# nh13/DWGSIM

Hardware: AMD Instinct MI355X
Metric: M read-pairs/sec (2x150 bp PE) (higher is better)
Workload: dtype u8

## Files before the change

### dwgsim_amd/api.py

```python
from __future__ import annotations
import ctypes as C
import os
import shlex
from dataclasses import dataclass, field

_HERE = os.path.dirname(os.path.abspath(__file__))
LIB_PATH = os.environ.get("DWGSIM_HIP_LIB") or os.path.join(_HERE, "libdwgsim_hip.so")

STREAM_BWA1, STREAM_BWA2, STREAM_BFAST = 0, 1, 2
STREAM_NAMES = {0: "bwa.read1.fastq", 1: "bwa.read2.fastq", 2: "bfast.fastq"}


class Params(C.Structure):
    _fields_ = [
        ("e_start", C.c_double * 2), ("e_end", C.c_double * 2),
        ("is_inner", C.c_int32), ("dist", C.c_int32), ("std_dev", C.c_double),
        ("N", C.c_int64), ("C", C.c_double), ("length", C.c_int32 * 2),
        ("mut_rate", C.c_double), ("mut_freq", C.c_double), ("indel_frac", C.c_double), ("indel_extend", C.c_double),
        ("indel_min", C.c_int32), ("rand_read", C.c_double), ("max_n", C.c_int32), ("data_type", C.c_int32),
        ("strandedness", C.c_int32), ("read_one_strand", C.c_int32), ("is_hap", C.c_int32), ("seed", C.c_int32),
        ("fixed_quality", C.c_int32), ("quality_std", C.c_double), ("reads_output_type", C.c_int32),
        ("output_type", C.c_int32), ("amplicons", C.c_int32), ("read_prefix", C.c_char_p), ("flow_order", C.c_char_p),
        ("use_base_error", C.c_int32),
    ]
# ... 165 lines not shown

def parse_flags(flags: str, lib=None) -> Params:
    p = default_params(lib)
    toks = shlex.split(flags)
    i = 0
    keep = []
    mut_input = None
    regions = None
    while i < len(toks):
        t = toks[i]
        def arg():
            nonlocal i
            i += 1
            return toks[i]
        if t == "-i": p.is_inner = 1
        elif t == "-d": p.dist = int(arg())
        elif t == "-s": p.std_dev = float(arg())
        elif t == "-N": p.N = int(arg()); p.C = -1
        elif t == "-C": p.C = float(arg()); p.N = -1
        elif t == "-1": p.length[0] = int(arg())
        elif t == "-2": p.length[1] = int(arg())
        elif t == "-e": p.e_start[0], p.e_end[0] = _error_rate(arg())
        elif t == "-E": p.e_start[1], p.e_end[1] = _error_rate(arg())
        elif t == "-r": p.mut_rate = float(arg())
        elif t == "-F": p.mut_freq = float(arg())
        elif t == "-R": p.indel_frac = float(arg())
        elif t == "-X": p.indel_extend = float(arg())
        elif t == "-I": p.indel_min = int(arg())
        elif t == "-c": p.data_type = int(arg())
        elif t == "-S": p.strandedness = int(arg())
        elif t == "-A": p.read_one_strand = int(arg())
        elif t == "-n": p.max_n = int(arg())
        elif t == "-y": p.rand_read = float(arg())
        elif t == "-f": keep.append(arg().encode()); p.flow_order = keep[-1]
        elif t == "-B": p.use_base_error = 1
        elif t == "-H": p.is_hap = 1
        elif t == "-z": p.seed = int(arg())
        elif t == "-M": p.output_type = int(arg())
        elif t == "-P": keep.append(arg().encode()); p.read_prefix = keep[-1]
        elif t == "-q": p.fixed_quality = ord(arg()[0])
        elif t == "-Q": p.quality_std = float(arg())
        elif t == "-o": p.reads_output_type = int(arg())
        elif t == "-a": p.amplicons = 1
        elif t == "-x": regions = arg()
        elif t in ("-m", "-b", "-v"): mut_input = ({"-b": 0, "-m": 1, "-v": 2}[t], arg())
        else:
            raise DwgsimError(f"option {t} is not on the accelerated path")
        i += 1
    p._keep = keep
    p._regions = regions
    p._mut_input = mut_input
    return p


def read_fasta(path: str):
    import numpy as np
    out = []
    name, chunks = None, []
    with open(path, "rb") as f:
        data = f.read()
    at = data.find(b">")
    while at >= 0:
        nl = data.find(b"\n", at)
        header = data[at + 1:] if nl < 0 else data[at + 1:nl]
        nxt = -1 if nl < 0 else data.find(b">", nl + 1)
        body = b"" if nl < 0 else (data[nl + 1:] if nxt < 0 else data[nl + 1:nxt])
        header = header.replace(b"\r", b"")
        name = header.split(b" ")[0].split(b"\t")[0].decode("latin-1")
        arr = np.frombuffer(body, dtype=np.uint8)
        keep = ((arr >= 65) & (arr <= 90)) | ((arr >= 97) & (arr <= 122)) | (arr == 45) | (arr == 46)
        out.append((name, np.ascontiguousarray(arr[keep])))
        at = nxt
    return out


@dataclass
class JobResult:
    streams: dict = field(default_factory=dict)
    mutations_txt: bytes = b""
    mutations_vcf: bytes = b""
    n_pairs: int = 0
    n_random: int = 0
    n_retries: int = 0
    kernel_ms: float = 0.0
    sim_kernel_ms: float = 0.0
    walk_ms: float = 0.0
    flow_cap_mult: int = 1


VCF_HEADER_POST = (
    b"##INFO=<ID=AF,Number=A,Type=Float,Description=\"Allele Frequency\">\n"
    b"##INFO=<ID=pl,Number=1,Type=Integer,Description=\"Phasing: 1 - HET contig 1, #2 - HET contig #2, 3 - HOM both contigs\">\n"
    b"##INFO=<ID=mt,Number=1,Type=String,Description=\"Variant Type: SUBSTITUTE/INSERT/DELETE\">\n"
    b"#CHROM\tPOS\tID\tREF\tALT\tQUAL\tFILTER\tINFO\n")


class Context:

    def __init__(self, params: Params, device: int = 0, lib=None):
        self.lib = lib or load()
        self.params = params
        err = C.c_int(0)
        self.h = self.lib.dwgsim_hip_create(C.byref(params), device, C.byref(err))
        if not self.h:
            raise DwgsimError(f"dwgsim_hip_create failed with code {err.value}" + (" (no HIP device? there is no CPU fallback)" if err.value == -2 else " (the library said why on stderr)"))
        for kv in os.environ.get("DWGSIM_HIP_DEBUG", "").split(","):
            if "=" in kv:
                self.lib.dwgsim_hip_debug_option(self.h, kv.split("=")[0].encode(), int(kv.split("=")[1]))

    def close(self):
        if self.h:
            self.lib.dwgsim_hip_destroy(self.h)
            self.h = None

    def __enter__(self):
        return self

    def __exit__(self, *a):
        self.close()

    def _chk(self, rc):
        if rc < 0:
            raise DwgsimError(f"error {rc}: {self.lib.dwgsim_hip_last_error(self.h).decode(errors='replace')}")
        return rc

    def add_contig(self, name: str, ascii_arr, contig_index: int) -> int:
        import numpy as np
        arr = np.ascontiguousarray(ascii_arr, dtype=np.uint8)
        return self._chk(self.lib.dwgsim_hip_add_contig(self.h, name.encode(), arr.ctypes.data_as(C.c_void_p), len(arr), contig_index))

    def drop_contig(self, cid: int):
        self._chk(self.lib.dwgsim_hip_drop_contig(self.h, cid))

    def add_contigs(self, contigs, first_index: int = 0, indices=None) -> int:
        import numpy as np
        n = len(contigs)
        arrs = [np.ascontiguousarray(a, dtype=np.uint8) for _, a in contigs]
        names = (C.c_char_p * n)(*[nm.encode() for nm, _ in contigs])
        ptrs = (C.c_void_p * n)(*[a.ctypes.data for a in arrs])
        lens = (C.c_int64 * n)(*[len(a) for a in arrs])
        idx = (C.c_uint32 * n)(*(indices if indices is not None else range(first_index, first_index + n)))
        return self._chk(self.lib.dwgsim_hip_add_contigs(self.h, n, names, ptrs, lens, idx))

    def mutate_async(self, cid: int):
        self._chk(self.lib.dwgsim_hip_mutate_async(self.h, cid))

    def mutate_wait(self, cid: int):
        self._chk(self.lib.dwgsim_hip_mutate_wait(self.h, cid))

    @staticmethod
    def _ranges(ranges):
        arr = (Range * len(ranges))()
        for k, (cid, first, n) in enumerate(ranges):
            arr[k].contig, arr[k].first_ii, arr[k].n_pairs = cid, first, n
        return arr

    def count_random_ranges(self, ranges, per_range: bool = False):
        n = C.c_uint64(0)
        per = (C.c_uint64 * len(ranges))() if per_range else None
        self._chk(self.lib.dwgsim_hip_count_random_ranges(self.h, self._ranges(ranges), len(ranges), C.byref(n), per))
        return list(per) if per_range else n.value

    def simulate_ranges_async(self, ranges, rand_base: int = RAND_CHAIN, slot: int = 0):
        self._chk(self.lib.dwgsim_hip_simulate_ranges_async(self.h, self._ranges(ranges), len(ranges), rand_base, slot))

    def simulate_ranges(self, ranges, rand_base: int, slot: int = 0) -> Batch:
# ... 150 lines not shown
            if have_regions and not last_takes_rest:
                l_eff = ctx.region_length(ci, arr)
                if l_eff < 0:
                    continue
            n_pairs = pairs_for_contig(params, l_eff, tot_len, n_ref == 0, n_sim, lib)
            if n_pairs < 0:
                continue
        n_sim += n_pairs
        yield ci, name, arr, n_pairs, l_eff


def split_ranges(ranges, batch_pairs):
    batch, room = [], batch_pairs
    for cid, first, n in ranges:
        while n > 0:
            take = min(n, room)
            batch.append((cid, first, take))
            first += take; n -= take; room -= take
            if room == 0:
                yield batch
                batch, room = [], batch_pairs
    if batch:
        yield batch


def run_job(params: Params, contigs, device: int = 0, batch_pairs: int = 1 << 22, fetch: bool = True, lib=None, debug_options=None, group_bp: int = 0, check_list_form: bool = False) -> JobResult:
    lib = lib or load()
    res = JobResult(streams={0: bytearray(), 1: bytearray(), 2: bytearray()})
    want_mut = params.output_type != 1
    want_reads = params.output_type != 2
    vcf = bytearray()
    txt = bytearray()
    if want_mut:
        vcf += b"##fileformat=VCFv4.1\n"
        for name, arr in contigs:
            vcf += f"##contig=<ID={name},length={len(arr)}>\n".encode()
        vcf += VCF_HEADER_POST
    n_sim = 0
    rand_ii = 0
    with Context(params, device, lib) as ctx:
        for k, v in (debug_options or {}).items():
            ctx.debug_option(k, v)
        if getattr(params, "_mut_input", None):
            ctx.set_mutation_input(params._mut_input[0], params._mut_input[1], contigs)
        have_regions = bool(getattr(params, "_regions", None))
        sched = list(schedule_contigs(params, contigs, ctx, lib))
        groups, cur, cur_bp = [], [], 0
        for ent in sched:
            if cur and (group_bp <= 0 or cur_bp + len(ent[2]) > group_bp):
                groups.append(cur); cur, cur_bp = [], 0
            cur.append(ent); cur_bp += len(ent[2])
        if cur:
            groups.append(cur)
        for grp in groups:
            h0 = ctx.add_contigs([(name, arr) for _, name, arr, _, _ in grp], indices=[ci for ci, _, _, _, _ in grp])
            if have_regions:
                for k, ent in enumerate(grp):
                    ctx.set_placement_length(h0 + k, ent[4])
            ctx.mutate(h0)
            if want_mut:
                for k in range(len(grp)):
                    t, v = ctx.mutations_text(h0 + k)
                    txt += t
                    vcf += v
                if check_list_form:
                    tv = ctx.mutations_via_list(h0)
                    if b"".join(a for a, _ in tv) != b"".join(ctx.mutations_text(h0 + k)[0] for k in range(len(grp))) or \
                       b"".join(b for _, b in tv) != b"".join(ctx.mutations_text(h0 + k)[1] for k in range(len(grp))):
                        raise DwgsimError("mutations_take / mutlist_text differs from mutations_text")
            ranges = [(h0 + k, 0, ent[3]) for k, ent in enumerate(grp) if want_reads and ent[3] > 0]
            for batch in split_ranges(ranges, batch_pairs):
                b = ctx.simulate_ranges(batch, rand_ii, 0)
                res.kernel_ms += b.kernel_ms
                res.sim_kernel_ms += b.sim_kernel_ms
                res.n_retries += b.n_retries
                if fetch:
                    for s in range(3):
                        if b.bytes[s]:
                            res.streams[s] += ctx.fetch(0, s, b.bytes[s])
                rand_ii += b.n_random
                n_sim += b.n_pairs
            ctx.drop_contig(h0)
        res.flow_cap_mult = ctx.debug_get("flow_cap_mult")
    res.n_pairs = n_sim
    res.n_random = rand_ii
    res.mutations_txt = bytes(txt)
    res.mutations_vcf = bytes(vcf)
    res.streams = {k: bytes(v) for k, v in res.streams.items()}
    return res


def run_job_api(params: Params, contigs, devices=None, gzip_on_gpu: bool = True, batch_pairs: int = 0, group_bp: int = 0, min_share: int = 0,
                lib=None, keep_output: bool = True, offset_sink: bool = False) -> JobResult:
    import gzip as _gz
    import numpy as np
    lib = lib or load()
    res = JobResult(streams={0: bytearray(), 1: bytearray(), 2: bytearray()})
    raw = {0: [], 1: [], 2: []}
    txt, vcf = bytearray(), bytearray()
    if params.output_type != 1:
        vcf += b"##fileformat=VCFv4.1\n"
        for name, arr in contigs:
            vcf += f"##contig=<ID={name},length={len(arr)}>\n".encode()
        vcf += VCF_HEADER_POST
    order = {"mut": [], "text_n": {0: 0, 1: 0, 2: 0}}

    def on_mut(user, name, t, tl, v, vl):
        order["mut"].append(name.decode())
        txt.extend(C.string_at(t, tl) if tl else b"")
        vcf.extend(C.string_at(v, vl) if vl else b"")
        return 0

    def on_reads(user, stream, data, n, text_n, gz):
        order["text_n"][stream] += text_n
        if keep_output:
            raw[stream].append((bool(gz), C.string_at(data, n), text_n))
        return 0

    import threading
    at_lock = threading.Lock(); at_pieces = {0: [], 1: [], 2: []}; at_threads = set()

    def on_reads_at(user, stream, offset, data, n, text_n, gz):
        blob = C.string_at(data, n) if keep_output else b""
        with at_lock:
            at_threads.add(threading.get_ident())
            order["text_n"][stream] += text_n
            at_pieces[stream].append((offset, n, bool(gz), blob, text_n))
        return 0

    sink = JobSink(None, MUT_CB(on_mut), READS_CB(on_reads), MSG_CB(lambda u, m: None), READS_AT_CB(on_reads_at) if offset_sink else READS_AT_CB())
    opt = JobOptions(1 if gzip_on_gpu else 0, 1, batch_pairs, group_bp, min_share)
    err = C.c_int(0)
    devs = (C.c_int * len(devices))(*devices) if devices else None
    job = lib.dwgsim_hip_job_create(C.byref(params), devs, len(devices) if devices else 0, C.byref(sink), C.byref(opt), C.byref(err))
    if not job:
        raise DwgsimError(f"dwgsim_hip_job_create failed with code {err.value}")
    try:
        def chk(rc):
            if rc < 0:
                raise DwgsimError(f"error {rc}: {lib.dwgsim_hip_job_last_error(job).decode(errors='replace')}")
        n = len(contigs)
        names = (C.c_char_p * n)(*[nm.encode() for nm, _ in contigs])
        lens = (C.c_int64 * n)(*[len(a) for _, a in contigs])
        chk(lib.dwgsim_hip_job_set_contig_table(job, names, lens, n))
        if getattr(params, "_regions", None):
            chk(lib.dwgsim_hip_job_set_regions(job, params._regions.encode()))
        if getattr(params, "_mut_input", None):
            chk(lib.dwgsim_hip_job_set_mutation_input(job, params._mut_input[0], params._mut_input[1].encode()))
        chk(lib.dwgsim_hip_job_prepare(job, None))
        for name, arr in contigs:
            a = np.ascontiguousarray(arr, dtype=np.uint8)
            r = lib.dwgsim_hip_job_add_contig(job, name.encode(), a.ctypes.data_as(C.c_void_p), len(a))
            if r < 0 and not is_skip(r):
                chk(r)
            if r > 0:
                res.n_pairs += r
        chk(lib.dwgsim_hip_job_finish(job))
    finally:
        lib.dwgsim_hip_job_destroy(job)
    if offset_sink:
        for s_ in range(3):
            at = 0
            for off, n, gz, blob, text_n in sorted(at_pieces[s_]):
                if off != at:
                    raise DwgsimError(f"reads_at: stream {s_} has a gap or an overlap at offset {at} (next piece at {off})")
                at += n
# ... 176 lines not shown
```

### dwgsim_amd/csrc/dw_host.cpp

```cpp
#include <hip/hip_runtime.h>
#include <math.h>
#include <stdio.h>
#include <stdlib.h>
#include <string.h>
#include <limits.h>
#include <ctype.h>
#include <stdarg.h>
#include <stdint.h>
#include <sys/mman.h>
#include <mutex>
#include <thread>
#include <string>
#include <vector>
#include <algorithm>
#include <array>
#include <stddef.h>
#include <type_traits>
#include "../../include/dwgsim_hip.h"
#include "dw_kernels.hpp"
#include "dw_launch.hpp"
#include "dw_mutin.hpp"
#include "dw_mem.hpp"

using namespace dw;

namespace {

struct HostIns { std::vector<int32_t> pos; std::vector<uint32_t> len, off; std::vector<uint8_t> bases; };

struct Member {
    std::string name;
    int64_t l = 0, l_place = 0;
    uint32_t contig_index = 0;
    int32_t start = 0;
    int32_t reg_off = 0, n_reg = 0;
    uint32_t name_off = 0; int32_t name_fixed_len = 0;
    ResolvedContig rc;
};

struct GroupMem {
    DevMem d_ref, d_cells[2], d_view[2];
    DevMem d_ins_pos[2], d_ins_len[2], d_ins_off[2], d_ins_bases[2];
    DevMem d_names, d_reg, d_seg;
    std::vector<uint8_t> h_names; std::vector<int32_t> h_reg, h_seg;
    DevMem d_summ[2], d_summ2[2];
    DevMem d_refview, d_refsumm, d_refsumm2, d_dirty;
    DevEvent ev_walk, ev_walk0;
    HostMem h_wc;
};

struct WalkCounters {
    uint64_t unused0[7];
    uint64_t n_cand;
    uint32_t max_del;
    struct { uint32_t entries, bases; } ins[2];
    uint32_t unused1;
    uint32_t slot_over;
    uint32_t n_cand_true;
    uint64_t mut_debug[2];
    uint64_t n_listed;
    uint64_t unused2;
};
static_assert(std::is_standard_layout<WalkCounters>::value && sizeof(WalkCounters) == 16 * 8, "the walk's counter block is 16 u64 words");
static_assert(offsetof(WalkCounters, n_cand) == 7 * 8 && offsetof(WalkCounters, max_del) == 8 * 8 && offsetof(WalkCounters, ins) == 8 * 8 + 4 && offsetof(WalkCounters, slot_over) == 8 * 8 + 6 * 4 &&
              offsetof(WalkCounters, n_cand_true) == 8 * 8 + 7 * 4 && offsetof(WalkCounters, mut_debug) == 12 * 8 && offsetof(WalkCounters, n_listed) == 14 * 8, "every counter at the word the kernels were given before the block had a type");
struct WcSpan { size_t off, bytes; };
#define WC_SPAN(first, last) WcSpan{offsetof(WalkCounters, first), offsetof(WalkCounters, last) + sizeof(WalkCounters::last) - offsetof(WalkCounters, first)}
constexpr WcSpan WC_RANDOM = WC_SPAN(n_cand, n_cand_true), WC_FILE = WC_SPAN(mut_debug, mut_debug), WC_LISTED = WC_SPAN(n_listed, n_listed);

struct Group {
    bool alive = false, mutated = false, walk_pending = false;
    int first_handle = -1;
    std::vector<Member> m;
    int64_t total = 0;
    GroupMem mem;
    uint32_t n_ins[2] = {0, 0}, n_ins_bases[2] = {0, 0};
    int fixed_max = 0;
    uint32_t n_cand = 0;
    bool dirty_any = false, dirty_all = false;
    int walk_attempt = 0; uint32_t walk_cap = 0; size_t walk_cap_bases = 0; bool walk_reset = false;
    uint32_t n_patch = 0, n_patch_ev = 0;
    bool list_valid = false; std::vector<int32_t> pos; std::vector<uint32_t> cells; HostIns ins[2];
};

struct HandleRef { int group = -1, k = 0; };

constexpr int N_COUNTERS = 32;

struct Counters {
    DevMem d; HostMem h;
    uint64_t *dev() const { return d.get<uint64_t>(); }
    uint64_t *host() const { return h.get<uint64_t>(); }
};

struct Slot {
    Counters counters;
    hipEvent_t ev_k0 = nullptr, ev_k1 = nullptr, ev_end = nullptr, ev_done = nullptr, ev_fetched = nullptr;
    bool pending = false, empty = true, fetch_in_flight = false;
    int group = -1;
    uint64_t n_pairs = 0, out_bytes[3] = {0, 0, 0}, gz_bytes[3] = {0, 0, 0};
    DevMem gz_out[3], gz_status, segs;
    HostMem h_segs;
    std::vector<dwgsim_hip_range_t> ranges;
    DevMem d_rerun_chain;
    int cap_mult = 1;
};

}

struct dwgsim_hip_ctx {
    dwgsim_hip_params_t prm;
    std::string read_prefix;
    std::vector<uint8_t> flow;
    DevMem d_flow;
    int device = 0;
    hipStream_t stream = nullptr;
    hipStream_t copy_stream = nullptr;
    hipStream_t walk_stream = nullptr;
    hipStream_t count_stream = nullptr;
    std::string err;
    double e_by[2] = {0, 0};
    DevMem d_thr[2];
    DevMem d_thr32[2]; int e_full = 0;
    DevMem d_qbase[2]; int32_t qb_words = 1;
    DevMem d_rand_fixed; int32_t rand_fixed_len = 0;
    std::vector<Group> groups;
    std::vector<GroupMem> pool;
    std::vector<HandleRef> handles;
    DevMem meta, fail_summ, block_rand, status_all, out[DWGSIM_HIP_SLOTS][3], split_state, split_hand, split_agg, split_pre, split_chunk;
    DevMem w_slots, w_slot_aux;
    int site_slots = -1; int64_t site_slot_cap = -1;
    DevMem scratch_mask, scratch_cnt, scratch_status, w_cand, w_ev, w_flags, w_lo, w_sufmin, w_bound, w_ppos, w_pcells, up_ascii, l_pos, l_cells, place_segs, place_rand, place_list, place_aux;
    HostMem h_up; hipEvent_t ev_up = nullptr; bool up_in_flight = false;
    HostMem h_place_segs, h_range_rand;
    std::vector<int32_t> h_ppos; std::vector<uint16_t> h_pcells; std::vector<Event> h_pev;
    bool seq_justify = false, dense_view = false;
    MutInput mutin; bool has_mutin = false;
    Regions regions; bool has_regions = false;
    DevMem flow_scratch, flow_free;
    Counters counters;
    DevMem d_wcounters;
    Counters pcounters;
    Slot slot[DWGSIM_HIP_SLOTS];
    DevMem d_chain;
    int chain_contig = -1; uint64_t chain_next_ii = 0;
    bool has_carry_override = false; uint64_t carry_override = 0;
    int flow_cap_forced = 0;
    int flow_cap_mult = 1;
    int ion_lds = -1;
    int n_cu = 0; int flow_slots = 0;
    int64_t walk_cap = -1; bool phases = false; int writer = -1, force_threads = 0; int64_t place_cap = -1; uint64_t place_open = 0; double walk_us = 0, count_us = 0; int split = -1;
    int64_t sim_form = 0;
    int64_t walk_form = 0;
    hipEvent_t ev_cnt0 = nullptr, ev_cnt1 = nullptr;
    bool gzip_on = false; DevMem d_crc_table, d_crc_shift;
    HostMem h_stage;
    std::string txt, vcf;
};

namespace {

#define HIPC(ctx, call) do { hipError_t e_ = (call); if (e_ != hipSuccess) { char b_[512]; snprintf(b_, sizeof b_, "HIP error %s at %s:%d (%s)", hipGetErrorString(e_), __FILE__, __LINE__, #call); (ctx)->err = b_; return DWGSIM_HIP_ERR_DEVICE; } } while (0)

hipError_t dev_malloc(dwgsim_hip_ctx *c, void **p, size_t bytes)
{
    hipError_t e = DevKind::alloc(p, bytes);
    if (e == hipSuccess || c->pool.empty()) return e;
    (void)hipGetLastError();
    hipStreamSynchronize(c->walk_stream);
    c->pool.clear();
    return DevKind::alloc(p, bytes);
}

hipError_t reserve(dwgsim_hip_ctx *c, DevMem &b, size_t need, size_t want)
{
    return b.reserve(need, want, [c](void **p, size_t n) { return dev_malloc(c, p, n); });
}

int ensure(dwgsim_hip_ctx *c, DevMem &b, size_t bytes)
{
    HIPC(c, reserve(c, b, bytes, bytes + bytes / 8 + 4096));
    return 0;
}

int upload(dwgsim_hip_ctx *c, DevMem &b, const void *src, size_t n)
{
    HIPC(c, reserve(c, b, n, n));
    const hipError_t e = hipMemcpy(b.get(), src, n, hipMemcpyHostToDevice);
    if (e != hipSuccess) b.reset();
    HIPC(c, e);
    return 0;
}

template <class T> int upload_table(dwgsim_hip_ctx_t *c, DevMem &d, const std::vector<T> &h, size_t slack)
{
    HIPC(c, reserve(c, d, sizeof(T) * h.size(), sizeof(T) * (h.size() + slack)));
    HIPC(c, hipMemcpyAsync(d.get(), h.data(), sizeof(T) * h.size(), hipMemcpyHostToDevice, c->walk_stream));
    return 0;
}

uint8_t nt4(int ch)
{
    switch (ch) { case 'A': case 'a': return 0; case 'C': case 'c': return 1; case 'G': case 'g': return 2; case 'T': case 't': return 3; case '-': return 5; default: return 4; }
}

void lazy_quality_params(double sigma, float *k, float *eps, float *lmin, int32_t *near1_zero)
{
    const double two_ln2 = 2.0 * log(2.0);
    double lm = 0.98 * (0.45 / sigma) * (0.45 / sigma) / two_ln2;
    if (!(lm < 0x1p-4)) lm = 0x1p-4;
    *near1_zero = lm >= 0x1p-10 ? 1 : 0;
    if (lm < 0x1p-10) lm = 0x1p-10;
    *lmin = (float)lm;
    lm = (double)*lmin * (1.0 - 0x1p-20);
    *k = (float)(sqrt(two_ln2) * sigma);
    *eps = (float)(1.5 * sigma * (3.4e-7 / sqrt(lm) + 7.2e-6) + 0x1p-18);
}

WalkParams walk_params(const dwgsim_hip_ctx *c)
{
    WalkParams w; w.mut_rate = c->prm.mut_rate; w.indel_frac = c->prm.indel_frac; w.indel_extend = c->prm.indel_extend;
    w.indel_min = c->prm.indel_min; w.is_hap = c->prm.is_hap; w.seed = (uint32_t)c->prm.seed;
    w.mut_thr = !(c->prm.mut_rate > 0) ? 0 : c->prm.mut_rate >= 1.0 ? 0x100000000ull : (uint64_t)ceil(c->prm.mut_rate * 4294967296.0);
    flow_gap_params(w.mut_thr, &w.gap_r, &w.gap_s);
    w.lg = reinterpret_cast<const uint32_t *>(c->d_flow.get() + 64);
    return w;
}

size_t padded_cells(const Group &g) { return (size_t)g.total + CELL_PAD; }

size_t view_bytes(size_t padded) { return padded / 2; }
size_t summ_bytes(size_t padded) { return sizeof(uint16_t) * (padded / SUMM_CELLS); }
size_t summ2_bytes(size_t padded) { return sizeof(uint16_t) * (padded / SUMM2_CELLS); }
uint32_t dirty_words(size_t padded) { return (uint32_t)((padded + 32 * SUMM_CELLS - 1) / (32 * SUMM_CELLS)); }
// ... 476 lines not shown
    const size_t view = view_bytes(padded) + 32, summ = summ_bytes(padded) + 32, summ2 = summ2_bytes(padded) + 32;
    const struct { DevMem *buf; size_t bytes; } cellbufs[] = {
        {&M.d_ref, padded}, {&M.d_cells[0], padded}, {&M.d_view[0], view}, {&M.d_summ[0], summ}, {&M.d_summ2[0], summ2},
        {&M.d_cells[1], padded}, {&M.d_view[1], view}, {&M.d_summ[1], summ}, {&M.d_summ2[1], summ2},
        {&M.d_refview, view}, {&M.d_refsumm, summ}, {&M.d_refsumm2, summ2}, {&M.d_dirty, dirty_bytes(padded)}};
    for (const auto &b : cellbufs) b.buf->reset();
    for (const auto &b : cellbufs) HIPC(c, reserve(c, *b.buf, b.bytes, b.bytes));
    return 0;
}

static int upload_sequence(dwgsim_hip_ctx_t *c, int n, const uint8_t *const *ascii, const int64_t *lens, const int64_t *starts, int64_t total, size_t padded, bool &must_wait)
{
    if (ensure(c, c->up_ascii, padded)) return DWGSIM_HIP_ERR_DEVICE;
    uint8_t *d_ascii = c->up_ascii.get();
    must_wait = true;
    bool laid_out = true;
    for (int k = 0; k < n && laid_out; ++k) if (lens[k] > 0 && ascii[k] != ascii[0] + starts[k]) laid_out = false;
    if (laid_out && n > 0 && ascii[0] && is_page_locked(ascii[0])) {
        HIPC(c, hipMemcpyAsync(d_ascii, ascii[0], (size_t)total, hipMemcpyHostToDevice, c->walk_stream));
        HIPC(c, hipMemsetAsync(d_ascii + total, 0, padded - (size_t)total, c->walk_stream));
        must_wait = false;
    } else if (n <= 8) {
        HIPC(c, hipMemsetAsync(d_ascii, 0, padded, c->walk_stream));
        for (int k = 0; k < n; ++k) if (lens[k] > 0) HIPC(c, hipMemcpyAsync(d_ascii + starts[k], ascii[k], (size_t)lens[k], hipMemcpyHostToDevice, c->walk_stream));
    } else {
        if (c->up_in_flight) { HIPC(c, hipEventSynchronize(c->ev_up)); c->up_in_flight = false; }
        HIPC(c, c->h_up.reserve((size_t)total, (size_t)total + (size_t)total / 4 + 4096));
        uint8_t *h_up = c->h_up.get();
        for (int k = 0; k < n; ++k) {
            const int64_t end = starts[k] + lens[k], next = k + 1 < n ? starts[k + 1] : total;
            if (lens[k] > 0) memcpy(h_up + starts[k], ascii[k], (size_t)lens[k]);
            memset(h_up + end, 0, (size_t)(next - end));
        }
        HIPC(c, hipMemcpyAsync(d_ascii, h_up, (size_t)total, hipMemcpyHostToDevice, c->walk_stream));
        HIPC(c, hipMemsetAsync(d_ascii + total, 0, padded - (size_t)total, c->walk_stream));
        HIPC(c, hipEventRecord(c->ev_up, c->walk_stream)); c->up_in_flight = true;
    }
    return 0;
}

static int make_pristine(dwgsim_hip_ctx_t *c, const Group &g)
{
    const GroupMem &M = g.mem;
    const int64_t n_cells = (int64_t)padded_cells(g) & ~(int64_t)15;
    uint8_t *ref = M.d_ref.get();
    launch_pack(c->walk_stream, c->up_ascii.get(), ref, M.d_cells[0].get(), M.d_cells[1].get(), n_cells);
    launch_make_view(c->walk_stream, ref, ref, n_cells, g.total, M.d_refview.get(), M.d_view[0].get(), M.d_refsumm.get<uint16_t>(), M.d_summ[0].get<uint16_t>(), M.d_refsumm2.get<uint16_t>(), M.d_summ2[0].get<uint16_t>());
    if (const int rc = restore_pristine(c, g, 1, R_VIEW | R_SUMM | R_SUMM2, c->walk_stream)) return rc;
    if (const int rc = clear_dirty(c, g, c->walk_stream)) return rc;
    HIPC(c, hipGetLastError());
    return 0;
}

static int upload_group_tables(dwgsim_hip_ctx_t *c, Group &g)
{
    GroupMem &M = g.mem;
    const int n = (int)g.m.size();
    M.h_seg.assign((size_t)(3 * n + 1), 0);
    for (int k = 0; k < n; ++k) { M.h_seg[(size_t)k] = g.m[(size_t)k].start; M.h_seg[(size_t)(n + 1 + k)] = (int32_t)g.m[(size_t)k].l; M.h_seg[(size_t)(2 * n + 1 + k)] = (int32_t)g.m[(size_t)k].contig_index; }
    M.h_seg[(size_t)n] = (int32_t)g.total;
    if (const int rc = upload_table(c, M.d_seg, M.h_seg, 64)) return rc;
    M.h_names.clear();
    for (Member &m : g.m) {
        const std::string nf = c->read_prefix.empty() ? m.name : c->read_prefix + "_" + m.name;
        m.name_fixed_len = (int32_t)nf.size(); m.name_off = (uint32_t)M.h_names.size();
        if (m.name_fixed_len > g.fixed_max) g.fixed_max = m.name_fixed_len;
        const size_t room = ((nf.size() + 1 < 256 ? 272 : nf.size() + 1 + 16) + 15) & ~(size_t)15;
        M.h_names.resize(M.h_names.size() + room, 0);
        M.h_names[m.name_off] = '@'; memcpy(&M.h_names[m.name_off + 1], nf.data(), nf.size());
    }
    if (const int rc = upload_table(c, M.d_names, M.h_names, 4096)) return rc;
    M.h_reg.clear();
    if (!c->has_regions) return 0;
    for (Member &m : g.m) {
        std::vector<int32_t> st, en; int64_t tot = 0;
        for (size_t q = 0; q < c->regions.contig.size(); ++q) if (c->regions.contig[q] == m.contig_index) { st.push_back((int32_t)c->regions.start[q]); en.push_back((int32_t)c->regions.end[q]); tot += c->regions.end[q] - c->regions.start[q]; }
        m.reg_off = (int32_t)M.h_reg.size(); m.n_reg = (int32_t)st.size(); m.l_place = tot;
        M.h_reg.insert(M.h_reg.end(), st.begin(), st.end()); M.h_reg.insert(M.h_reg.end(), en.begin(), en.end());
    }
    M.h_reg.push_back(0);
    return upload_table(c, M.d_reg, M.h_reg, 64);
}

static int build_group(dwgsim_hip_ctx_t *c, Group &g, const uint8_t *const *ascii, const int64_t *lens, const int64_t *starts)
{
    const int n = (int)g.m.size();
    const size_t padded = padded_cells(g);
    bool must_wait = true;
    if (const int rc = reserve_cell_buffers(c, g.mem, padded)) return rc;
    if (const int rc = upload_sequence(c, n, ascii, lens, starts, g.total, padded, must_wait)) return rc;
    if (const int rc = make_pristine(c, g)) return rc;
    if (const int rc = upload_group_tables(c, g)) return rc;
    if (c->has_mutin) for (int k = 0; k < n; ++k) resolve_mutation_input(c->mutin, g.m[(size_t)k].contig_index, ascii[k], lens[k], (uint32_t)c->prm.seed, c->prm.is_hap != 0, g.m[(size_t)k].rc);
    if (must_wait) HIPC(c, hipStreamSynchronize(c->walk_stream));
    return 0;
}

int dwgsim_hip_add_contigs(dwgsim_hip_ctx_t *c, int n, const char *const *names, const uint8_t *const *ascii, const int64_t *lens, const uint32_t *contig_index)
{
    if (!c || n < 1 || !names || !ascii || !lens || !contig_index) { if (c) c->err = "bad contig arguments"; return DWGSIM_HIP_ERR_ARG; }
    for (int k = 0; k < n; ++k) if (!names[k] || (!ascii[k] && lens[k] > 0) || lens[k] < 0 || lens[k] > INT32_MAX) { c->err = "bad contig arguments"; return DWGSIM_HIP_ERR_ARG; }
    std::vector<int64_t> starts((size_t)n);
    const int64_t total = dwgsim_hip_group_layout(lens, n, starts.data());
    if (total < 0 || total > (int64_t)INT32_MAX - 2 * GROUP_ALIGN) { c->err = "dwgsim-hip: the contigs of one group must stay below 2^31 cells in all (add them in smaller groups)\n"; return DWGSIM_HIP_ERR_ARG; }
    HIPC(c, hipSetDevice(c->device));
    const int gid = take_group(c, (size_t)total + CELL_PAD);
    Group &g = c->groups[(size_t)gid];
    g.alive = true; g.total = total; g.first_handle = (int)c->handles.size();
    g.m.resize((size_t)n);
    for (int k = 0; k < n; ++k) { Member &m = g.m[(size_t)k]; m.name = names[k]; m.l = m.l_place = lens[k]; m.contig_index = contig_index[k]; m.start = (int32_t)starts[(size_t)k]; }
    const int rc = build_group(c, g, ascii, lens, starts.data());
    if (rc != 0) { (void)hipStreamSynchronize(c->walk_stream); g = Group(); return rc; }
    for (int k = 0; k < n; ++k) c->handles.push_back(HandleRef{gid, k});
    return g.first_handle;
}

int dwgsim_hip_add_contig(dwgsim_hip_ctx_t *c, const char *name, const uint8_t *ascii, int64_t len, uint32_t contig_index)
{
    return dwgsim_hip_add_contigs(c, 1, &name, &ascii, &len, &contig_index);
}

int dwgsim_hip_drop_contig(dwgsim_hip_ctx_t *c, int contig)
{
    Group *g = get_group(c, contig);
    if (!g) return DWGSIM_HIP_ERR_ARG;
    hipSetDevice(c->device);
    const int gid = (int)(g - c->groups.data());
    for (int s = 0; s < DWGSIM_HIP_SLOTS; ++s) if (c->slot[s].pending && !c->slot[s].empty && c->slot[s].group == gid) { c->err = "drop_contig: a batch that reads this group has not been waited for (dwgsim_hip_wait first)"; return DWGSIM_HIP_ERR_STATE; }
    if (g->walk_pending) hipEventSynchronize(g->mem.ev_walk.get());
    for (size_t k = 0; k < g->m.size(); ++k) { if (c->chain_contig == g->first_handle + (int)k) c->chain_contig = -1; c->handles[(size_t)g->first_handle + k].group = -1; }
    c->pool.push_back(std::move(g->mem));
    *g = Group();
    if (c->pool.size() > 3) {
        hipStreamSynchronize(c->walk_stream);
        c->pool.erase(c->pool.begin());
    }
    return DWGSIM_HIP_OK;
}

int dwgsim_hip_set_regions(dwgsim_hip_ctx_t *c, const char *path, const char *const *names, const int64_t *lens, int n_contigs, uint64_t *total_len)
{
    if (!c || !path || n_contigs < 0 || (n_contigs && (!names || !lens))) { if (c) c->err = "bad regions arguments"; return DWGSIM_HIP_ERR_ARG; }
    if (c->prm.amplicons) { c->err = "Error: cannot use a regions BED file (-x) when simulating amplicons (-a)\n"; return DWGSIM_HIP_ERR_ARG; }
    std::vector<ContigName> tab;
    for (int i = 0; i < n_contigs; ++i) tab.push_back(ContigName{names[i], lens[i]});
    std::string err;
    if (!parse_regions(path, tab, c->regions, err)) { c->err = err; c->has_regions = false; return DWGSIM_HIP_ERR_ARG; }
    c->has_regions = true;
    uint64_t tot = 0;
    for (size_t q = 0; q < c->regions.start.size(); ++q) tot += c->regions.end[q] - c->regions.start[q];
    if (total_len) *total_len = tot;
    return DWGSIM_HIP_OK;
}

int64_t dwgsim_hip_contig_region_length(dwgsim_hip_ctx_t *c, uint32_t contig_index, const uint8_t *ascii, int64_t len, int64_t *non_acgt, int64_t *region_bases)
{
    if (non_acgt) *non_acgt = 0;
    if (region_bases) *region_bases = len;
    if (!c || !c->has_regions) return len;
    int64_t m = 0, num_n = 0;
    for (size_t q = 0; q < c->regions.contig.size(); ++q) if (c->regions.contig[q] == contig_index) {
        m += c->regions.end[q] - c->regions.start[q];
        for (int64_t p = c->regions.start[q]; p <= (int64_t)c->regions.end[q]; ++p) { const int ch = (p >= 1 && p - 1 < len) ? ascii[p - 1] : 'N'; if (nt4(ch) >= 4) ++num_n; }
    }
    if (non_acgt) *non_acgt = num_n;
    if (region_bases) *region_bases = m;
    if (m == 0) return DWGSIM_HIP_SKIP_NO_REGION;
    if (0.95 < num_n / (double)m) return DWGSIM_HIP_SKIP_NON_ACGT;
    return m;
}

int dwgsim_hip_contig_set_placement_length(dwgsim_hip_ctx_t *c, int contig, int64_t l)
{
    int k = 0;
    Group *g = get_group(c, contig, &k);
// ... 79 lines not shown
        HIPC(c, hipMemcpyAsync(c->w_pcells.get(), c->h_pcells.data(), sizeof(uint16_t) * np, hipMemcpyHostToDevice, st));
        if (nev) HIPC(c, hipMemcpyAsync(c->w_ev.get(), c->h_pev.data(), sizeof(Event) * nev, hipMemcpyHostToDevice, st));
        launch_apply_patches(st, c->w_ppos.get<int32_t>(), c->w_pcells.get<uint16_t>(), np, M.d_cells[0].get(), M.d_cells[1].get());
        launch_mut_debug(st, M.d_ref.get(), M.d_cells[0].get(), M.d_cells[1].get(), g.total, &wc->mut_debug[0]);
        if (nev) justify(c, st, c->w_ev.get<Event>(), Count{nullptr, nev}, group_dev(g));
        launch_mut_debug(st, M.d_ref.get(), M.d_cells[0].get(), M.d_cells[1].get(), g.total, &wc->mut_debug[1]);
    }
    make_views(st, g);
    g.dirty_all = true;
    HIPC(c, hipGetLastError());
    HIPC(c, wc_fetch(c, M, WC_FILE, st));
    HIPC(c, hipEventRecord(M.ev_walk.get(), st));
    return DWGSIM_HIP_OK;
}

enum class Restore { None, Chunks, All };
struct WalkPlan {
    uint32_t cap; size_t ncap, cap_bases;
    uint32_t nblk;
    bool use_slots; uint32_t nbs, slot_cap; size_t slot_bytes;
    Restore restore;
    bool dense;
};

static WalkPlan walk_plan(const dwgsim_hip_ctx_t *c, const Group &g)
{
    WalkPlan P;
    P.cap = g.walk_cap; P.ncap = P.cap ? P.cap : 1; P.cap_bases = g.walk_cap_bases;
    P.nblk = (uint32_t)((g.total + SCAN_POS_PER_BLOCK - 1) / SCAN_POS_PER_BLOCK);
    P.nbs = site_scan_blocks(g.total);
    const double m = (double)site_scan_block_positions() * (c->prm.mut_rate > 0 ? c->prm.mut_rate : 0.0);
    P.slot_cap = (uint32_t)std::min<double>((double)site_scan_block_positions(), m + 8.0 * sqrt(m + 1.0) + 32.0);
    if (c->site_slot_cap >= 0) P.slot_cap = (uint32_t)std::max<int64_t>(1, c->site_slot_cap);
    P.slot_bytes = (size_t)P.nbs * P.slot_cap * sizeof(int32_t);
    P.use_slots = g.walk_attempt == 0 && c->site_slots != 0 && P.nbs > 0 && (c->site_slots > 0 || P.slot_bytes <= std::max<size_t>((size_t)64 << 20, P.ncap * 16));
    P.restore = g.walk_attempt > 0 || g.dirty_all ? Restore::All : g.dirty_any ? Restore::Chunks : Restore::None;
    P.dense = c->seq_justify || c->dense_view;
    return P;
}

static int walk_reserve(dwgsim_hip_ctx_t *c, Group &g, const WalkPlan &P)
{
    if (ensure(c, c->scratch_status, ((size_t)P.nblk + 2) * sizeof(uint64_t)) ||
        ensure(c, c->w_cand, sizeof(int32_t) * P.ncap) || ensure(c, c->w_ev, sizeof(Event) * P.ncap) ||
        ensure(c, c->w_flags, sizeof(uint4) * (P.ncap + 64)) ||
        ensure(c, c->w_lo, sizeof(int32_t) * P.ncap) || ensure(c, c->w_sufmin, sizeof(int32_t) * (P.ncap + 64)) ||
        ensure(c, c->w_bound, P.ncap)) return DWGSIM_HIP_ERR_DEVICE;
    for (int h = 0; h < 2; ++h) if (const int rc = ensure_ins(c, g, h, P.ncap, P.cap_bases)) return rc;
    if (P.use_slots && (ensure(c, c->w_slots, P.slot_bytes) || ensure(c, c->w_slot_aux, 2 * (size_t)P.nbs * sizeof(uint32_t)))) return DWGSIM_HIP_ERR_DEVICE;
    return DWGSIM_HIP_OK;
}

static int walk_launch(dwgsim_hip_ctx_t *c, Group &g, const WalkPlan &P)
{
    hipStream_t st = c->walk_stream;
    const WalkParams wp = walk_params(c);
    const SegTab seg = seg_tab(g);
    const GroupMem &M = g.mem;
    WalkCounters *wc = c->d_wcounters.get<WalkCounters>();
    int32_t *d_cand = c->w_cand.get<int32_t>(); Event *d_ev = c->w_ev.get<Event>(); uint4 *d_flags = c->w_flags.get<uint4>();
    uint32_t *tot4 = &wc->ins[0].entries;
    const Count nc{&wc->n_cand, P.cap};
    HIPC(c, wc_fill(c, WC_RANDOM, 0, st));
    if (P.use_slots) launch_site_scan_slots(st, M.d_refview.get(), g.total, seg, wp, c->w_slots.get<int32_t>(), P.slot_cap, c->w_slot_aux.get<uint32_t>(), d_cand, P.cap, &wc->n_cand, &wc->slot_over);
    else {
        uint64_t *d_status = c->scratch_status.get<uint64_t>();
        HIPC(c, hipMemsetAsync(d_status, 0, ((size_t)P.nblk + 2) * sizeof(uint64_t), st));
        launch_site_scan_list(st, M.d_refview.get(), g.total, seg, wp, d_status, d_status + P.nblk, d_cand, P.cap, &wc->n_cand);
    }
    launch_events(st, d_cand, nc, M.d_ref.get(), seg, wp, d_ev, &wc->max_del);
    launch_resolve(st, d_ev, nc, &wc->max_del, d_flags, tot4);
    ContigDev cd = group_dev(g);
    cd.tot4 = tot4; cd.cap_bases[0] = (uint32_t)std::min<size_t>(ins_bases_cap(g, 0), 0xFFFFFFFFu); cd.cap_bases[1] = (uint32_t)std::min<size_t>(ins_bases_cap(g, 1), 0xFFFFFFFFu);
    launch_apply(st, d_ev, nc, d_flags, cd, wp);
    justify(c, st, d_ev, nc, cd);
    if (P.dense) {
        make_views(st, g);
        g.dirty_all = true;
    } else {
        launch_mark_dirty(st, d_ev, nc, c->w_lo.get<int32_t>(), M.d_dirty.get<uint32_t>());
        dirty_chunks(st, false, g);
        g.dirty_any = true;
    }
    HIPC(c, hipGetLastError());
    return DWGSIM_HIP_OK;
}

static int walk_random(dwgsim_hip_ctx_t *c, Group &g)
{
    const WalkPlan P = walk_plan(c, g);
    if (const int rc = walk_reserve(c, g, P)) return rc;
    c->walk_form = pack_walk_form(g.walk_attempt, false, P.use_slots, (int)P.restore, P.dense);
    hipStream_t st = c->walk_stream;
    HIPC(c, hipEventRecord(g.mem.ev_walk0.get(), st));
    if (P.restore == Restore::All) { for (int h = 0; h < 2; ++h) if (const int rc = restore_pristine(c, g, h, R_ALL, st)) return rc; }
    else if (P.restore == Restore::Chunks) dirty_chunks(st, true, g);
    if (P.restore != Restore::None) { if (const int rc = clear_dirty(c, g, st)) return rc; g.dirty_all = g.dirty_any = false; }
    if (const int rc = walk_launch(c, g, P)) return rc;
    HIPC(c, wc_fetch(c, g.mem, WC_RANDOM, st));
    HIPC(c, hipEventRecord(g.mem.ev_walk.get(), st));
    return DWGSIM_HIP_OK;
}

static void collect_file_mutations(dwgsim_hip_ctx_t *c, const Group &g, HostIns (&hi)[2])
{
    c->h_ppos.clear(); c->h_pcells.clear(); c->h_pev.clear();
    for (size_t k = 0; k < g.m.size(); ++k) {
        const Member &m = g.m[k];
        for (size_t q = 0; q < m.rc.pos.size(); ++q) {
            c->h_ppos.push_back(m.rc.pos[q] + m.start); c->h_pcells.push_back(m.rc.cells[q]);
            if (m.rc.cells[q] & 0x3030) { Event e; e.pos = m.rc.pos[q] + m.start; e.type = 4; e.hap = 3; e.base = 0; e.live = 1; e.len = 1; e.seg = (uint32_t)k; c->h_pev.push_back(e); }
        }
        for (int h = 0; h < 2; ++h) for (const InsPayload &ip : m.rc.ins[h]) {
            hi[h].pos.push_back(ip.pos + m.start); hi[h].len.push_back((uint32_t)ip.bases.size()); hi[h].off.push_back((uint32_t)hi[h].bases.size());
            hi[h].bases.insert(hi[h].bases.end(), ip.bases.begin(), ip.bases.end());
        }
    }
}

static int upload_ins_tables(dwgsim_hip_ctx_t *c, Group &g, HostIns (&hi)[2])
{
    for (int h = 0; h < 2; ++h) {
        const size_t n = hi[h].pos.size(), nb = hi[h].bases.size();
        g.n_ins[h] = (uint32_t)n; g.n_ins_bases[h] = (uint32_t)nb;
        if (const int rc = ensure_ins(c, g, h, n ? n : 1, nb ? nb : 1)) return rc;
        if (n) for (const InsTable &t : ins_tables(g.mem, h, hi[h])) HIPC(c, hipMemcpy(t.dev, t.host, t.bytes, hipMemcpyHostToDevice));
    }
    return DWGSIM_HIP_OK;
}

static void initial_walk_caps(const dwgsim_hip_ctx_t *c, Group &g)
{
    double mean = 0;
    for (const Member &m : g.m) mean += (double)m.l * c->prm.mut_rate;
    g.walk_cap = (uint32_t)std::min<double>((double)g.total, mean + 8.0 * sqrt(mean + 1.0) + 256.0);
    g.walk_cap_bases = (size_t)g.walk_cap * 8 + 4096;
    if (c->walk_cap >= 0) { g.walk_cap = (uint32_t)c->walk_cap; g.walk_cap_bases = 1; }
}

int dwgsim_hip_mutate_async(dwgsim_hip_ctx_t *c, int contig)
{
    Group *gp = get_group(c, contig);
    if (!gp) return DWGSIM_HIP_ERR_ARG;
    Group &g = *gp;
    if (g.walk_pending) { c->err = "mutate: the group's previous walk was not waited for"; return DWGSIM_HIP_ERR_STATE; }
    for (const Slot &sl : c->slot) if (sl.pending && sl.group == c->handles[(size_t)contig].group) { c->err = "mutate: a batch that reads this group is still in flight (wait for it first)"; return DWGSIM_HIP_ERR_STATE; }
    HIPC(c, hipSetDevice(c->device));
    g.walk_reset = g.mutated;
    for (int h = 0; h < 2; ++h) g.n_ins[h] = g.n_ins_bases[h] = 0;
    g.mutated = true; g.n_cand = 0; g.list_valid = false;
    g.walk_attempt = 0;
    if (g.total == 0) return DWGSIM_HIP_OK;
    if (c->has_mutin) {
        HIPC(c, hipStreamSynchronize(c->walk_stream));
        HostIns hi[2];
        collect_file_mutations(c, g, hi);
        g.n_patch = (uint32_t)c->h_ppos.size(); g.n_patch_ev = (uint32_t)c->h_pev.size();
        g.n_cand = g.n_patch_ev;
        HIPC(c, hipStreamSynchronize(c->walk_stream));
        if (const int rc = upload_ins_tables(c, g, hi)) return rc;
    } else initial_walk_caps(c, g);
    if (const int rc = c->has_mutin ? walk_file_driven(c, g) : walk_random(c, g)) return rc;
    g.walk_pending = true;
    return DWGSIM_HIP_OK;
}

// ... 189 lines not shown
    if (const int rc = fetch_mutated_list(c, g)) return rc;
    const Member &m = g.m[(size_t)km];
    format_mutations(ListView{g.pos.data(), g.cells.data(), g.pos.size(), g.ins}, m.name, m.start, m.l, c->txt, c->vcf);
    if (txt) *txt = c->txt.data();
    if (txt_len) *txt_len = c->txt.size();
    if (vcf) *vcf = c->vcf.data();
    if (vcf_len) *vcf_len = c->vcf.size();
    return DWGSIM_HIP_OK;
}

struct dwgsim_hip_mutlist {
    std::vector<int32_t> pos; std::vector<uint32_t> cells; HostIns ins[2];
    struct M { std::string name; int64_t l; int32_t start; };
    std::vector<M> m;
    std::string txt, vcf;
};

dwgsim_hip_mutlist_t *dwgsim_hip_mutations_take(dwgsim_hip_ctx_t *c, int contig, int *n_contigs)
{
    if (n_contigs) *n_contigs = 0;
    if (!c) return nullptr;
    Group *gp = get_group(c, contig);
    if (!gp) return nullptr;
    Group &g = *gp;
    if (!g.mutated || g.walk_pending) { c->err = "mutate_contig must run first"; return nullptr; }
    if (hipSetDevice(c->device) != hipSuccess) { c->err = "mutations_take: device error"; return nullptr; }
    if (fetch_mutated_list(c, g)) return nullptr;
    auto *L = new dwgsim_hip_mutlist();
    L->pos.swap(g.pos); L->cells.swap(g.cells);
    for (int h = 0; h < 2; ++h) { L->ins[h] = std::move(g.ins[h]); g.ins[h] = HostIns(); }
    g.list_valid = false;
    for (const Member &m : g.m) L->m.push_back({m.name, m.l, m.start});
    if (n_contigs) *n_contigs = (int)L->m.size();
    return L;
}

int dwgsim_hip_mutlist_text(dwgsim_hip_mutlist_t *L, int k, const char **txt, size_t *txt_len, const char **vcf, size_t *vcf_len)
{
    if (!L || k < 0 || k >= (int)L->m.size()) return DWGSIM_HIP_ERR_ARG;
    const auto &m = L->m[(size_t)k];
    format_mutations(ListView{L->pos.data(), L->cells.data(), L->pos.size(), L->ins}, m.name, m.start, m.l, L->txt, L->vcf);
    if (txt) *txt = L->txt.data();
    if (txt_len) *txt_len = L->txt.size();
    if (vcf) *vcf = L->vcf.data();
    if (vcf_len) *vcf_len = L->vcf.size();
    return DWGSIM_HIP_OK;
}

void dwgsim_hip_mutlist_free(dwgsim_hip_mutlist_t *L) { delete L; }

namespace {
struct Launch { SimForm f; SimArgs a; Group *g = nullptr; std::vector<SimSeg> segs; uint64_t n_pairs = 0; uint32_t nblk = 0; int fixed_max = 0; };
struct SimPlan {
    size_t cap[3];
    int32_t lb_shift; bool too_many;
    size_t block_rand, status, meta, fail_summ, split_state, split_hand, split_agg, split_pre, split_chunk;
    bool scratch; int32_t flow_slots; size_t flow_scratch, flow_free;
    size_t segs, gz_chunks[3], gz_cap[3], gz_status;
};
struct ChainSet { uint64_t *words; int set_rand, set_carry; uint64_t carry; };
}

static int build_ranges(dwgsim_hip_ctx_t *c, const dwgsim_hip_range_t *r, int n, uint64_t ppb, Launch &L)
{
    if (!r || n < 1) { c->err = "bad range arguments"; return DWGSIM_HIP_ERR_ARG; }
    Group *g = nullptr;
    uint64_t pairs = 0, blocks = 0; int fmax = 0;
    std::vector<SimSeg> &segs = L.segs;
    segs.clear();
    for (int q = 0; q < n; ++q) {
        int k = 0;
        Group *gq = get_group(c, r[q].contig, &k);
        if (!gq) return DWGSIM_HIP_ERR_ARG;
        if (g && gq != g) { c->err = "the ranges of one call must belong to contigs that were added together (dwgsim_hip_add_contigs)"; return DWGSIM_HIP_ERR_ARG; }
        g = gq;
        if (r[q].n_pairs == 0) continue;
        const Member &m = g->m[(size_t)k];
        if (c->has_regions && m.n_reg == 0 && c->prm.rand_read < 1.0) { c->err = "dwgsim-hip: this contig has no target region (-x): the reference's placement loop would not terminate\n"; return DWGSIM_HIP_ERR_ARG; }
        SimSeg s; memset(&s, 0, sizeof s);
        s.first_block = (uint32_t)blocks; s.contig_index = m.contig_index; s.start = m.start; s.l = (int32_t)m.l;
        s.first_ii = r[q].first_ii; s.n_pairs = r[q].n_pairs; s.pair_off = pairs; s.l_place = m.l_place;
        s.reg_off = m.reg_off; s.n_reg = m.n_reg; s.name_off = m.name_off; s.name_fixed_len = m.name_fixed_len;
        s.contig_start = r[q].first_ii == 0 ? 1u : 0u;
        segs.push_back(s);
        pairs += r[q].n_pairs; blocks += (r[q].n_pairs + ppb - 1) / ppb;
        if (m.name_fixed_len > fmax) fmax = m.name_fixed_len;
        if (blocks > 0x7fffffffull) { c->err = "too many pairs in one call"; return DWGSIM_HIP_ERR_ARG; }
    }
    if (!g->mutated || g->walk_pending) { c->err = "mutate_contig must run first"; return DWGSIM_HIP_ERR_STATE; }
    L.g = g; L.n_pairs = pairs; L.nblk = (uint32_t)blocks; L.fixed_max = fmax;
    return DWGSIM_HIP_OK;
}

static int sim_form(dwgsim_hip_ctx_t *c, SimForm &f)
{
    const dwgsim_hip_params_t &p = c->prm;
    const size_t qb = (size_t)c->qb_words;
    const int lmax = p.length[0] > p.length[1] ? p.length[0] : p.length[1];
    f = SimForm();
    f.lpp = p.length[1] > 0 ? 2 : 1;
    f.out = (p.reads_output_type != 2 ? 1 : 0) | (p.reads_output_type != 1 ? 2 : 0);
    f.dt = p.data_type;
    f.nthr = SIM_THREADS;
    f.cap = lmax; f.lds_words = (lmax + 7) / 8;
    bool fifo = true;
    if (p.data_type == 0) {
        const int cap_fifo = 5, cap_reg = (p.reads_output_type == 0) ? 4 : 5;
        const int b_fifo = sim_blocks_per_cu(sim_lds_bytes((size_t)f.lds_words, SIM_THREADS, qb, true), cap_fifo), b_reg = sim_blocks_per_cu(sim_lds_bytes((size_t)f.lds_words, SIM_THREADS, qb, false), cap_reg);
        if (b_fifo < b_reg && !(p.reads_output_type == 0 && b_fifo >= 3)) fifo = false;
        if (c->writer >= 0) fifo = c->writer != 0;
    }
    const size_t need = sim_lds_bytes((size_t)f.lds_words, SIM_THREADS, qb, fifo);
    if (p.data_type != 2 && (need > SIM_LDS_BUDGET || ((sim_blocks_per_cu(need, 8) < 2 || c->force_threads == SIM_THREADS_LONG) && c->force_threads != SIM_THREADS))) {
        f.nthr = SIM_THREADS_LONG; fifo = true;
        if (sim_lds_bytes(0, SIM_THREADS_LONG, qb, true) > SIM_LDS_BUDGET) {
            char b[160]; snprintf(b, sizeof b, "dwgsim-hip: reads longer than %d bases are not supported for -c 0 / -c 1\n", (int)((SIM_LDS_BUDGET - SIM_THREADS_LONG * SIM_FIFO_BYTES) / 2 - 16));
            c->err = b; return DWGSIM_HIP_ERR_UNSUP;
        }
    }
    if (p.data_type == 2) {
        f.cap = std::max(flow_base_capacity(c), lmax) * c->flow_cap_mult;
        f.lds_words = (f.cap + 15) / 16; f.cap = 16 * f.lds_words;
        f.stack_words = std::min(FLOW_STACK_WORDS * c->flow_cap_mult, FLOW_STACK_WORDS_MAX);
        const size_t per_lane = (size_t)(f.lds_words + f.stack_words);
        const size_t need256 = sim_lds_bytes(per_lane, SIM_THREADS, qb, true), need64 = sim_lds_bytes(per_lane, ION_THREADS_SMALL, qb, true);
        int mode = c->ion_lds;
        if (mode < 0) mode = (need256 <= SIM_LDS_BUDGET && sim_blocks_per_cu(need256, 8) >= 2) ? 1 : (need64 <= SIM_LDS_BUDGET && sim_blocks_per_cu(need64, 32) >= 4) ? 2 : 0;
        if ((mode == 1 && need256 > SIM_LDS_BUDGET) || (mode == 2 && need64 > SIM_LDS_BUDGET)) mode = 0;
        f.dt = mode != 0 ? 3 : 2; f.nthr = mode == 2 ? ION_THREADS_SMALL : SIM_THREADS;
    }
    const bool split_wins = lmax <= 50;
    f.split = (p.data_type == 0 && f.nthr == SIM_THREADS && (c->split < 0 ? split_wins : c->split != 0)) ? 1 : 0;
    if (f.dt == 3 && f.nthr == SIM_THREADS && f.cap < 32768 && c->split != 0) f.split = 1;
    if (f.split && c->writer < 0) fifo = true;
    const size_t stage = f.dt == 3 ? (size_t)(f.lds_words + f.stack_words) : f.dt == 2 ? (size_t)f.stack_words : f.nthr != SIM_THREADS ? 0 : (size_t)f.lds_words;
    if (f.split) { f.wr = fifo ? 2 : 0; f.lds = sim_lds_bytes(stage, (size_t)f.nthr, 0, false); f.lds_b = sim_lds_bytes(0, (size_t)f.nthr, qb, fifo, SIM_FIFO_BYTES_WIDE); }
    else { f.wr = fifo ? 1 : 0; f.lds = sim_lds_bytes(stage, (size_t)f.nthr, qb, fifo); }
    return 0;
}

static void fill_sim_args(const dwgsim_hip_ctx_t *c, const Group &g, const SimForm &f, SimArgs &a)
{
    const dwgsim_hip_params_t &p = c->prm;
    memset(&a, 0, sizeof a);
    a.p.std_dev = p.std_dev; a.p.mut_freq = p.mut_freq; a.p.rand_read = p.rand_read; a.p.quality_std = p.quality_std;
    a.p.dist = p.dist; a.p.is_inner = p.is_inner; a.p.len[0] = p.length[0]; a.p.len[1] = p.length[1]; a.p.max_n = p.max_n;
    a.p.strandedness = p.strandedness; a.p.read_one_strand = p.read_one_strand; a.p.amplicons = p.amplicons;
    a.p.fixed_quality = p.fixed_quality; a.p.data_type = p.data_type;
    a.p.has_bfast = p.reads_output_type != 1; a.p.has_bwa = p.reads_output_type != 2;
    a.p.seed = (uint32_t)p.seed;
    lazy_quality_params(p.quality_std, &a.p.q_k, &a.p.q_eps, &a.p.q_lmin, &a.p.q_near1);
    fill_haps(g, a.hap);
    a.chain = c->d_chain.get<uint64_t>();
    a.have_regions = c->has_regions ? 1 : 0; a.reg = g.mem.d_reg.get<int32_t>();
    for (int j = 0; j < 2; ++j) { a.e_thr[j] = c->d_thr[j].get<uint64_t>(); a.e_thr32[j] = c->d_thr32[j].get<uint32_t>(); a.qbase[j] = c->d_qbase[j].get<uint32_t>() ? c->d_qbase[j].get<uint32_t>() : c->d_qbase[0].get<uint32_t>(); }
    a.qb_words = c->qb_words;
    a.e_full = c->e_full;
    a.names = g.mem.d_names.get();
    a.summ[0] = g.mem.d_summ[0].get<uint16_t>(); a.summ[1] = g.mem.d_summ[1].get<uint16_t>(); a.summ2[0] = g.mem.d_summ2[0].get<uint16_t>(); a.summ2[1] = g.mem.d_summ2[1].get<uint16_t>();
    a.place_fast = (!c->has_regions && !p.amplicons && p.std_dev * 12.1 + 2.0 < 1e9) ? 1 : 0;
    a.place_k = a.place_fast ? (int32_t)ceil(p.std_dev * 12.1) + 2 : 0;
    a.rand_fixed = c->d_rand_fixed.get(); a.rand_fixed_len = c->rand_fixed_len;
    a.sim_threads = f.nthr; a.fifo = f.wr != 0; a.split = f.split; a.ion_lds = f.dt == 3;
    a.cap = f.cap; a.lds_words = f.lds_words; a.flow_stack_words = f.stack_words;
    a.flow = c->d_flow.get(); a.flow_len = (int32_t)c->flow.size();
    for (int j = 0; j < 2; ++j) {
        const int n = c->prm.length[j];
        uint64_t tmax = 0, tmin = ~0ull;
        for (int i = 0; i < n; ++i) {
            const double ei = c->prm.e_start[j] + c->e_by[j] * i;
            const uint64_t t = !(ei > 0) ? 0 : ei >= 1.0 ? 0x100000000ull : (uint64_t)ceil(ei * 4294967296.0);
            tmax = std::max(tmax, t); tmin = std::min(tmin, t);
        }
        a.err_thr_max[j] = n > 0 ? tmax : 0; a.err_ramp[j] = (n > 0 && tmin != tmax) ? 1 : 0;
        flow_gap_params(a.err_thr_max[j], &a.err_gap_r[j], &a.err_gap_s[j]);
    }
    for (int j = 0; j < 2; ++j) {
        const double e0 = c->prm.e_start[j];
        flow_gap_params(!(e0 > 0) ? 0 : e0 >= 1.0 ? 0x100000000ull : (uint64_t)ceil(e0 * 4294967296.0), &a.flow_gap_r[j], &a.flow_gap_s[j]);
    }
}

static int sim_resolve(dwgsim_hip_ctx_t *c, const dwgsim_hip_range_t *r, int n, Launch &L)
{
    if (!r || n < 1) { c->err = "bad range arguments"; return DWGSIM_HIP_ERR_ARG; }
    if (!get_group(c, r[0].contig)) return DWGSIM_HIP_ERR_ARG;
    if (const int rc = sim_form(c, L.f)) return rc;
    if (const int rc = build_ranges(c, r, n, (uint64_t)(L.f.nthr / L.f.lpp), L)) return rc;
    fill_sim_args(c, *L.g, L.f, L.a);
    return DWGSIM_HIP_OK;
}

int dwgsim_hip_count_random_ranges(dwgsim_hip_ctx_t *c, const dwgsim_hip_range_t *r, int n, uint64_t *n_random, uint64_t *per_range)
{
    if (!c) return DWGSIM_HIP_ERR_ARG;
    if (n_random) *n_random = 0;
    if (per_range) for (int q = 0; q < n; ++q) per_range[q] = 0;
    Launch L;
    if (const int rc = build_ranges(c, r, n, PLACE_PAIRS, L)) return rc;
    const uint64_t n_pairs = L.n_pairs; const uint32_t n_blocks = L.nblk;
    if (n_pairs == 0) return DWGSIM_HIP_OK;
    Group &g = *L.g;
    HIPC(c, hipSetDevice(c->device));
    hipStream_t st = c->count_stream;
    if (g.walk_pending) { if (const int rc = dwgsim_hip_mutate_wait(c, g.first_handle)) return rc; }
    if (g.mem.ev_walk.get() && g.mutated) HIPC(c, hipStreamWaitEvent(st, g.mem.ev_walk.get(), 0));
    if (const int rc = sim_form(c, L.f)) return rc;
    SimArgs &a = L.a; fill_sim_args(c, g, L.f, a);
    const size_t ns = L.segs.size();
    if (ensure(c, c->place_rand, sizeof(uint32_t) * ((size_t)n_blocks + 1)) || ensure(c, c->place_segs, sizeof(SimSeg) * ns) ||
        ensure(c, c->place_aux, PLACE_LISTS * 16 * sizeof(uint32_t) + sizeof(uint64_t) * ns)) return DWGSIM_HIP_ERR_DEVICE;
    if (sizeof(SimSeg) * ns > c->h_place_segs.cap() || sizeof(uint64_t) * ns > c->h_range_rand.cap()) HIPC(c, hipStreamSynchronize(st));
    HIPC(c, c->h_place_segs.reserve(sizeof(SimSeg) * ns, sizeof(SimSeg) * (ns + 64))); HIPC(c, c->h_range_rand.reserve(sizeof(uint64_t) * ns, sizeof(uint64_t) * (ns + 64)));
    const uint64_t *h_range_rand = c->h_range_rand.get<uint64_t>();
    memcpy(c->h_place_segs.get(), L.segs.data(), sizeof(SimSeg) * ns);
    HIPC(c, hipMemcpyAsync(c->place_segs.get(), c->h_place_segs.get(), sizeof(SimSeg) * ns, hipMemcpyHostToDevice, st));
    a.segs = c->place_segs.get<SimSeg>(); a.n_seg = (int32_t)ns; a.n_blocks = n_blocks; a.n_pairs = n_pairs;
    a.block_rand = c->place_rand.get<uint32_t>(); a.counters = c->pcounters.dev();
    const uint64_t waves = (uint64_t)n_blocks * (PLACE_PAIRS / 64);
    const uint32_t cap_full = (uint32_t)((waves + PLACE_LISTS - 1) / PLACE_LISTS) * 64u;
    uint32_t cap = (uint32_t)std::min<uint64_t>(cap_full, 1024 + n_pairs / PLACE_LISTS / 8);
    if (c->place_cap >= 0 && (uint64_t)c->place_cap < cap) cap = (uint32_t)c->place_cap;
    for (int attempt = 0;; ++attempt) {
        if (ensure(c, c->place_list, sizeof(uint32_t) * (size_t)cap * PLACE_LISTS)) return DWGSIM_HIP_ERR_DEVICE;
        a.place_list = c->place_list.get<uint32_t>(); a.place_list_cap = cap;
        a.place_list_n = c->place_aux.get<uint32_t>(); a.range_rand = reinterpret_cast<uint64_t *>(c->place_aux.get<uint8_t>() + PLACE_LISTS * 16 * sizeof(uint32_t));
        HIPC(c, hipMemsetAsync(c->pcounters.dev(), 0, N_COUNTERS * sizeof(uint64_t), st));
        HIPC(c, hipMemsetAsync(c->place_aux.get(), 0, PLACE_LISTS * 16 * sizeof(uint32_t) + sizeof(uint64_t) * ns, st));
        HIPC(c, hipEventRecord(c->ev_cnt0, st));
        launch_place(st, a);
        HIPC(c, hipEventRecord(c->ev_cnt1, st));
        HIPC(c, hipGetLastError());
        HIPC(c, hipMemcpyAsync(c->pcounters.host(), c->pcounters.dev(), N_COUNTERS * sizeof(uint64_t), hipMemcpyDeviceToHost, st));
        HIPC(c, hipMemcpyAsync(c->h_range_rand.get(), a.range_rand, sizeof(uint64_t) * ns, hipMemcpyDeviceToHost, st));
        HIPC(c, hipStreamSynchronize(st));
        { float ms = 0; if (hipEventElapsedTime(&ms, c->ev_cnt0, c->ev_cnt1) == hipSuccess) c->count_us += 1e3 * ms; else (void)hipGetLastError(); }
        if (!(c->pcounters.host()[2] & 16) || attempt > 0) break;
        cap = cap_full;
    }
    if (c->pcounters.host()[2] & 16) { c->err = "count_random: the list of undecided pairs overflowed twice"; return DWGSIM_HIP_ERR_FAILED; }
    if (c->pcounters.host()[2]) { char b[128]; snprintf(b, sizeof b, "\r[dwgsim_core] failed to generate a read after %d trials\n", MAX_ATTEMPTS + 1); c->err = b; return DWGSIM_HIP_ERR_FAILED; }
    c->place_open = c->pcounters.host()[5];
// ... 101 lines not shown
    for (int j = 0; j < 4; ++j) a.status[j] = f.split ? nullptr : c->status_all.get<uint64_t>() + (size_t)j * (size_t)nblk;
    if (f.split) { a.split_state = c->split_state.get<uint32_t>(); a.split_hand = c->split_hand.get<uint32_t>(); a.split_agg = c->split_agg.get<uint32_t>(); a.split_pre = c->split_pre.get<uint64_t>(); a.split_chunk = c->split_chunk.get<uint64_t>(); }
    if (P.scratch) { a.flow_scratch = c->flow_scratch.get<uint32_t>(); a.flow_free = c->flow_free.get<uint64_t>(); a.flow_slots = P.flow_slots; }
    sl.group = c->handles[(size_t)L.g->first_handle].group;
    launch_init(c->stream, sl.counters.dev(), (uint32_t)N_COUNTERS, a.status[0], f.split ? 0 : 4 * (uint64_t)nblk, a.flow_free, a.flow_free ? 256 + 8 * (uint64_t)nblk : 0,
                ch.words, rand_base, ch.set_rand, ch.carry, ch.set_carry);
    HIPC(c, hipEventRecord(sl.ev_k0, c->stream));
    c->sim_form = (int64_t)f.nthr << 20 | f.lpp << 16 | f.out << 12 | f.dt << 8 | f.wr << 4 | f.split;
    if (!launch_simulate(c->stream, a, f)) { c->err = "simulate: no k_simulate instance for this form"; return DWGSIM_HIP_ERR_FAILED; }
    HIPC(c, hipEventRecord(sl.ev_k1, c->stream));
    sl.cap_mult = c->flow_cap_mult;
    if (!rerun) launch_failrule(c->stream, a.meta, n_pairs, opens, c->fail_summ.get<uint64_t>(), sl.counters.dev(), c->d_chain.get<uint64_t>());
    if (c->gzip_on) {
        HIPC(c, hipMemsetAsync(sl.gz_status.get(), 0, P.gz_status, c->stream));
        size_t off = 0;
        for (int t = 0; t < 3; ++t) {
            if (P.cap[t] == 0) continue;
            launch_gzip(c->stream, a.out[t], &sl.counters.dev()[4 + t], P.cap[t], sl.gz_out[t].get<uint8_t>(), P.gz_cap[t], sl.gz_status.get<uint64_t>() + off, &sl.counters.dev()[28 + t], &sl.counters.dev()[24 + t], &sl.counters.dev()[2],
                        c->d_crc_table.get<uint32_t>(), c->d_crc_shift.get<uint32_t>());
            off += P.gz_chunks[t];
        }
    }
    HIPC(c, hipEventRecord(sl.ev_end, c->stream));
    HIPC(c, hipGetLastError());
    HIPC(c, hipMemcpyAsync(sl.counters.host(), sl.counters.dev(), N_COUNTERS * sizeof(uint64_t), hipMemcpyDeviceToHost, c->stream));
    HIPC(c, hipEventRecord(sl.ev_done, c->stream));
    sl.pending = true;
    return DWGSIM_HIP_OK;
}

static int sim_enqueue(dwgsim_hip_ctx_t *c, const dwgsim_hip_range_t *r, int n, uint64_t rand_base, int slot, bool rerun)
{
    if (!c || slot < 0 || slot >= DWGSIM_HIP_SLOTS) { if (c) c->err = "bad simulate arguments"; return DWGSIM_HIP_ERR_ARG; }
    if (c->slot[slot].pending) { c->err = "simulate: the slot still holds a batch that was not waited for"; return DWGSIM_HIP_ERR_STATE; }
    Launch L;
    if (const int rc = sim_resolve(c, r, n, L)) return rc;
    HIPC(c, hipSetDevice(c->device));
    const SimPlan P = sim_plan(c, L);
    if (P.too_many) { c->err = "too many pairs in one call"; return DWGSIM_HIP_ERR_ARG; }
    if (L.n_pairs) { if (const int rc = sim_reserve(c, slot, P)) return rc; }
    return sim_launch(c, slot, L, P, sim_chain(c, c->slot[slot], r, n, rand_base != DWGSIM_HIP_RAND_CHAIN, rerun), rand_base, rerun);
}

int dwgsim_hip_simulate_ranges_async(dwgsim_hip_ctx_t *c, const dwgsim_hip_range_t *r, int n, uint64_t rand_base, int slot) { return sim_enqueue(c, r, n, rand_base, slot, false); }

int dwgsim_hip_simulate_async(dwgsim_hip_ctx_t *c, int contig, uint64_t first_ii, uint64_t n_pairs, uint64_t rand_base, int slot)
{
    dwgsim_hip_range_t r; memset(&r, 0, sizeof r); r.contig = contig; r.first_ii = first_ii; r.n_pairs = n_pairs;
    return dwgsim_hip_simulate_ranges_async(c, &r, 1, rand_base, slot);
}

int dwgsim_hip_wait(dwgsim_hip_ctx_t *c, int slot, dwgsim_hip_batch_t *out)
{
    if (!c || slot < 0 || slot >= DWGSIM_HIP_SLOTS) { if (c) c->err = "bad slot"; return DWGSIM_HIP_ERR_ARG; }
    Slot &sl = c->slot[slot];
    if (out) memset(out, 0, sizeof *out);
    if (sl.empty) { sl.pending = false; return DWGSIM_HIP_OK; }
    if (!sl.pending) { c->err = "wait: no batch was enqueued on this slot"; return DWGSIM_HIP_ERR_STATE; }
    HIPC(c, hipSetDevice(c->device));
    HIPC(c, hipEventSynchronize(sl.ev_done));
    sl.pending = false;
    uint64_t *h = sl.counters.host();
    if ((h[2] & 2) && !(h[2] & ~(2ull | 8ull)) && c->prm.data_type == 2) {
        uint64_t keep[8]; for (int q = 0; q < 6; ++q) keep[q] = h[16 + q];
        const uint64_t base = h[22];
        while (h[2] & 2) {
            if (sl.cap_mult >= c->flow_cap_mult) {
                if ((int64_t)flow_base_capacity(c) * (int64_t)c->flow_cap_mult * 2 > (int64_t)FLOW_CAP_MAX) break;
                c->flow_cap_mult *= 2;
            }
            if (const int rc = sim_enqueue(c, sl.ranges.data(), (int)sl.ranges.size(), base, slot, true)) return rc;
            HIPC(c, hipEventSynchronize(sl.ev_done));
            sl.pending = false;
        }
        for (int q = 0; q < 6; ++q) h[16 + q] = keep[q];
    }
    if (h[2] & 4) { c->err = "dwgsim-hip: no fragment placement satisfied the target regions (-x) after 2^20 tries (the reference would not terminate)\n"; return DWGSIM_HIP_ERR_FAILED; }
    if (h[2] & 2) { c->err = "dwgsim-hip: a read outgrew its buffer (or degenerated) in the flow-error model\n"; return DWGSIM_HIP_ERR_FAILED; }
    if ((h[2] & ~8ull) || h[20]) {
        char b[128]; snprintf(b, sizeof b, "\r[dwgsim_core] failed to generate a read after %d trials\n", MAX_ATTEMPTS + 1); c->err = b; return DWGSIM_HIP_ERR_FAILED;
    }
    if (h[2] & 8) { c->err = "dwgsim-hip: the gzip output buffer is too small for this text\n"; return DWGSIM_HIP_ERR_FAILED; }
    for (int t = 0; t < 3; ++t) { sl.out_bytes[t] = h[4 + t]; sl.gz_bytes[t] = h[24 + t]; }
    if (c->phases) {
        uint64_t tot = 0; for (int k = 0; k < 8; ++k) tot += h[8 + k];
        fprintf(stderr, "[phases]");
        for (int k = 0; k < 8; ++k) fprintf(stderr, " p%d=%.1f%%", k, tot ? 100.0 * h[8 + k] / tot : 0.0);
        fprintf(stderr, " (ticks %llu)\n", (unsigned long long)tot);
    }
    if (out) {
        out->n_pairs = sl.n_pairs; out->n_random = h[3]; out->n_retries = h[1];
        for (int t = 0; t < 3; ++t) { out->bytes[t] = sl.out_bytes[t]; out->dev_ptr[t] = c->out[slot][t].get(); }
        for (int t = 0; t < 3; ++t) out->gz_bytes[t] = sl.gz_bytes[t];
        for (int t = 0; t < 4; ++t) out->fail_seg[t] = h[16 + t];
        out->fail_carry = h[21];
        HIPC(c, hipEventElapsedTime(&out->sim_kernel_ms, sl.ev_k0, sl.ev_k1));
        HIPC(c, hipEventElapsedTime(&out->kernel_ms, sl.ev_k0, sl.ev_end));
    }
    return DWGSIM_HIP_OK;
}

int dwgsim_hip_simulate(dwgsim_hip_ctx_t *c, int contig, uint64_t first_ii, uint64_t n_pairs, uint64_t rand_base, int slot, dwgsim_hip_batch_t *out)
{
    if (out) memset(out, 0, sizeof *out);
    const int rc = dwgsim_hip_simulate_async(c, contig, first_ii, n_pairs, rand_base, slot);
    if (rc != DWGSIM_HIP_OK) return rc;
    return dwgsim_hip_wait(c, slot, out);
}

namespace {
struct HostRegion { uint8_t *base; size_t len; };
std::mutex g_host_m;
std::vector<HostRegion> g_host;
}
static bool in_host_registry(const void *p)
{
    std::lock_guard<std::mutex> lk(g_host_m);
    for (const HostRegion &r : g_host) if ((const uint8_t *)p >= r.base && (const uint8_t *)p < r.base + r.len) return true;
    return false;
}
void *dwgsim_hip_host_alloc(size_t bytes)
{
    const size_t H = (size_t)2 << 20;
    const size_t len = ((bytes ? bytes : 1) + H - 1) / H * H;
    uint8_t *raw = (uint8_t *)mmap(nullptr, len + H, PROT_READ | PROT_WRITE, MAP_PRIVATE | MAP_ANONYMOUS, -1, 0);
    if (raw == MAP_FAILED) return nullptr;
    uint8_t *p = (uint8_t *)(((uintptr_t)raw + H - 1) & ~(uintptr_t)(H - 1));
    if (p > raw) munmap(raw, (size_t)(p - raw));
    if (p + len < raw + len + H) munmap(p + len, (size_t)(raw + len + H - (p + len)));
    (void)madvise(p, len, MADV_HUGEPAGE);
    auto touch = [p](size_t from, size_t upto) { for (size_t o = from; o < upto; o += 4096) ((volatile uint8_t *)p)[o] = 0; };
    const int nt = len >= ((size_t)64 << 20) ? 4 : 1;
    if (nt == 1) touch(0, len);
    else {
        std::vector<std::thread> th; const size_t per = (len / H + (size_t)nt - 1) / (size_t)nt * H;
        for (int k = 0; k < nt; ++k) { const size_t a = std::min(len, (size_t)k * per), b = std::min(len, a + per); if (b > a) th.emplace_back(touch, a, b); }
        for (auto &t : th) t.join();
    }
    if (hipHostRegister(p, len, hipHostRegisterDefault) != hipSuccess) { (void)hipGetLastError(); munmap(p, len); return nullptr; }
    { std::lock_guard<std::mutex> lk(g_host_m); g_host.push_back(HostRegion{p, len}); }
    return p;
}
void dwgsim_hip_host_free(void *p)
{
    if (!p) return;
    HostRegion r{nullptr, 0};
    {
        std::lock_guard<std::mutex> lk(g_host_m);
        for (size_t i = 0; i < g_host.size(); ++i) if (g_host[i].base == (uint8_t *)p) { r = g_host[i]; g_host.erase(g_host.begin() + (long)i); break; }
    }
    if (!r.base) return;
    (void)hipHostUnregister(r.base);
    munmap(r.base, r.len);
}

static int fetch_async(dwgsim_hip_ctx_t *c, int slot, int stream, void *host_dst, size_t cap, bool gz)
{
    if (!c || slot < 0 || slot >= DWGSIM_HIP_SLOTS || stream < 0 || stream > 2 || (!host_dst && cap)) { if (c) c->err = "bad fetch arguments"; return DWGSIM_HIP_ERR_ARG; }
    Slot &sl = c->slot[slot];
    if (sl.pending) { c->err = "fetch: wait for the batch first (its sizes are not known yet)"; return DWGSIM_HIP_ERR_STATE; }
    HIPC(c, hipSetDevice(c->device));
    const size_t n = (size_t)(gz ? sl.gz_bytes[stream] : sl.out_bytes[stream]);
    if (n > cap) { c->err = "fetch: destination too small"; return DWGSIM_HIP_ERR_ARG; }
    if (n == 0) return DWGSIM_HIP_OK;
    HIPC(c, hipMemcpyAsync(host_dst, gz ? sl.gz_out[stream].get() : c->out[slot][stream].get(), n, hipMemcpyDeviceToHost, c->copy_stream));
    HIPC(c, hipEventRecord(sl.ev_fetched, c->copy_stream));
// ... 37 lines not shown
    const size_t n = (size_t)sl.out_bytes[stream];
    if (n > cap) { c->err = "fetch: destination too small"; return DWGSIM_HIP_ERR_ARG; }
    if (n == 0) return DWGSIM_HIP_OK;
    if (is_page_locked(host_dst)) {
        HIPC(c, hipMemcpyAsync(host_dst, c->out[slot][stream].get(), n, hipMemcpyDeviceToHost, c->copy_stream));
        HIPC(c, hipStreamSynchronize(c->copy_stream));
        return DWGSIM_HIP_OK;
    }
    const size_t CH = (size_t)16 << 20;
    HIPC(c, c->h_stage.reserve(2 * CH, 2 * CH));
    const uint8_t *src = c->out[slot][stream].get<uint8_t>();
    uint8_t *stage[2] = {c->h_stage.get<uint8_t>(), c->h_stage.get<uint8_t>() + CH};
    size_t done = 0; int b = 0;
    size_t cur = n < CH ? n : CH;
    HIPC(c, hipMemcpyAsync(stage[0], src, cur, hipMemcpyDeviceToHost, c->copy_stream));
    while (done < n) {
        HIPC(c, hipStreamSynchronize(c->copy_stream));
        const size_t next_off = done + cur, next = next_off < n ? ((n - next_off) < CH ? (n - next_off) : CH) : 0;
        if (next) HIPC(c, hipMemcpyAsync(stage[b ^ 1], src + next_off, next, hipMemcpyDeviceToHost, c->copy_stream));
        memcpy((uint8_t *)host_dst + done, stage[b], cur);
        done += cur; cur = next; b ^= 1;
    }
    return DWGSIM_HIP_OK;
}

int dwgsim_hip_debug_count_byte(dwgsim_hip_ctx_t *c, int slot, int stream, int byte, uint64_t *count)
{
    if (!c || slot < 0 || slot >= DWGSIM_HIP_SLOTS || stream < 0 || stream > 2 || !count) return DWGSIM_HIP_ERR_ARG;
    HIPC(c, hipSetDevice(c->device));
    Slot &sl = c->slot[slot];
    if (sl.pending) { c->err = "count_byte: wait for the batch first"; return DWGSIM_HIP_ERR_STATE; }
    HIPC(c, hipMemsetAsync(&c->counters.dev()[15], 0, sizeof(uint64_t), c->stream));
    if (sl.out_bytes[stream]) launch_count_byte(c->stream, c->out[slot][stream].get<uint8_t>(), sl.out_bytes[stream], (uint32_t)(byte & 0xff), &c->counters.dev()[15]);
    HIPC(c, hipMemcpyAsync(&c->counters.host()[15], &c->counters.dev()[15], sizeof(uint64_t), hipMemcpyDeviceToHost, c->stream));
    HIPC(c, hipStreamSynchronize(c->stream));
    *count = c->counters.host()[15];
    return DWGSIM_HIP_OK;
}

int dwgsim_hip_debug_gzip(dwgsim_hip_ctx_t *c, const void *text, size_t n, void *out, size_t cap, size_t *out_n)
{
    if (!c || (!text && n) || !out_n) return DWGSIM_HIP_ERR_ARG;
    HIPC(c, hipSetDevice(c->device));
    if (const int rc = dwgsim_hip_set_gzip(c, c->gzip_on ? 1 : 0); rc < 0) return rc;
    if (!c->d_crc_shift) { const bool was = c->gzip_on; if (const int rc = dwgsim_hip_set_gzip(c, 1); rc < 0) return rc; c->gzip_on = was; }
    *out_n = 0;
    if (n == 0) return DWGSIM_HIP_OK;
    const size_t gcap = (size_t)gz_capacity(n), nch = (size_t)gz_chunks(n);
    DevMem text_m, out_m, aux_m;
    if (reserve(c, text_m, n + 64, n + 64) != hipSuccess || reserve(c, out_m, gcap + 64, gcap + 64) != hipSuccess || reserve(c, aux_m, sizeof(uint64_t) * (4 + nch), sizeof(uint64_t) * (4 + nch)) != hipSuccess) { c->err = "out of device memory"; return DWGSIM_HIP_ERR_DEVICE; }
    uint8_t *d_text = text_m.get(), *d_out = out_m.get(); uint64_t *d_aux = aux_m.get<uint64_t>();
    const uint64_t n64 = n;
    bool ok = hipMemcpyAsync(d_text, text, n, hipMemcpyHostToDevice, c->stream) == hipSuccess && hipMemsetAsync(d_aux, 0, sizeof(uint64_t) * (4 + nch), c->stream) == hipSuccess &&
              hipMemcpyAsync(d_aux, &n64, sizeof n64, hipMemcpyHostToDevice, c->stream) == hipSuccess;
    if (ok) {
        launch_gzip(c->stream, d_text, &d_aux[0], n, d_out, gcap, &d_aux[4], &d_aux[1], &d_aux[2], &d_aux[3], c->d_crc_table.get<uint32_t>(), c->d_crc_shift.get<uint32_t>());
        uint64_t res[4] = {0, 0, 0, 0};
        ok = hipGetLastError() == hipSuccess && hipMemcpyAsync(res, d_aux, sizeof res, hipMemcpyDeviceToHost, c->stream) == hipSuccess && hipStreamSynchronize(c->stream) == hipSuccess;
        if (ok && (res[3] & 8)) { c->err = "dwgsim-hip: the gzip output buffer is too small for this text\n"; return DWGSIM_HIP_ERR_FAILED; }
        if (ok && res[2] > cap) { c->err = "debug_gzip: destination too small"; return DWGSIM_HIP_ERR_ARG; }
        if (ok) { ok = hipMemcpy(out, d_out, (size_t)res[2], hipMemcpyDeviceToHost) == hipSuccess; *out_n = (size_t)res[2]; }
    }
    if (!ok) { c->err = "debug_gzip: device error"; return DWGSIM_HIP_ERR_DEVICE; }
    return DWGSIM_HIP_OK;
}

int dwgsim_hip_debug_option(dwgsim_hip_ctx_t *c, const char *key, int64_t value)
{
    if (!c || !key) return DWGSIM_HIP_ERR_ARG;
    if (!strcmp(key, "justify_seq")) c->seq_justify = value != 0;
    else if (!strcmp(key, "dense_view")) c->dense_view = value != 0;
    else if (!strcmp(key, "walk_cap")) c->walk_cap = value;
    else if (!strcmp(key, "site_slots")) c->site_slots = (int)value;
    else if (!strcmp(key, "site_slot_cap")) c->site_slot_cap = value;
    else if (!strcmp(key, "phases")) c->phases = value != 0;
    else if (!strcmp(key, "writer")) c->writer = (int)value;
    else if (!strcmp(key, "sim_threads")) c->force_threads = (int)value;
    else if (!strcmp(key, "walk_seg_min")) walk_debug_seg_min((uint32_t)value);
    else if (!strcmp(key, "place_cap")) c->place_cap = value;
    else if (!strcmp(key, "split")) c->split = (int)value;
    else if (!strcmp(key, "flow_slots")) c->flow_slots = (int)value;
    else if (!strcmp(key, "ion_lds")) c->ion_lds = (int)value;
    else if (!strcmp(key, "flow_cap")) c->flow_cap_forced = (int)value;
    else { c->err = "unknown debug option"; return DWGSIM_HIP_ERR_ARG; }
    return DWGSIM_HIP_OK;
}

int dwgsim_hip_debug_get(dwgsim_hip_ctx_t *c, const char *key, int64_t *value)
{
    if (!c || !key || !value) return DWGSIM_HIP_ERR_ARG;
    if (!strcmp(key, "place_open")) *value = (int64_t)c->place_open;
    else if (!strcmp(key, "flow_cap_mult")) *value = (int64_t)c->flow_cap_mult;
    else if (!strcmp(key, "walk_us")) *value = (int64_t)c->walk_us;
    else if (!strcmp(key, "count_us")) *value = (int64_t)c->count_us;
    else if (!strcmp(key, "sim_form")) *value = c->sim_form;
    else if (!strcmp(key, "walk_form")) *value = c->walk_form;
    else { c->err = "unknown debug value"; return DWGSIM_HIP_ERR_ARG; }
    return DWGSIM_HIP_OK;
}

}
```

### dwgsim_amd/csrc/dw_kernels.hpp

```cpp
#pragma once
#include <stdint.h>

namespace dw {

constexpr int PAIRS_PER_BLOCK = 128;
constexpr int PLACE_PAIRS = 256;
constexpr int PLACE_LISTS = 64;
#ifndef DW_SIM_THREADS
#define DW_SIM_THREADS 256
#endif
constexpr int SIM_THREADS = DW_SIM_THREADS;
constexpr int FLOW_STACK_WORDS = 4;
constexpr uint32_t FLOW_NEVER = 0xFFFFFFFFu;
constexpr int FLOW_LG_ENTRIES = 257;
constexpr int FLOW_CAP_MAX = 1 << 20;
constexpr int FLOW_STACK_WORDS_MAX = 32;
#ifndef DW_ION_THREADS_SMALL
#define DW_ION_THREADS_SMALL 128
#endif
constexpr int ION_THREADS_SMALL = DW_ION_THREADS_SMALL;
constexpr int SIM_THREADS_LONG = 64;
constexpr int SIM_FIFO_BYTES = 40;
constexpr int SIM_FIFO_BYTES_WIDE = 72;
inline size_t sim_lds_bytes(size_t words_per_lane, size_t lanes, size_t qb_words, bool fifo, size_t fifo_bytes = SIM_FIFO_BYTES) { return ((words_per_lane * lanes + 2 * qb_words + 3) & ~(size_t)3) * 4 + (fifo ? lanes * fifo_bytes : 0); }
inline int sim_blocks_per_cu(size_t dyn_lds, int cap) { const size_t per = (dyn_lds + 1700 + 1279) / 1280 * 1280;       const int b = (int)(163840 / per); return b < cap ? b : cap; }
constexpr size_t SIM_LDS_BUDGET = 150 * 1024;
struct SimForm {
    int lpp, out, dt, nthr, wr, split;
    size_t lds, lds_b;
    int cap, lds_words, stack_words;
};
constexpr int SCAN_POS_PER_THREAD = 16;
constexpr int SCAN_THREADS = 256;
constexpr int SCAN_POS_PER_BLOCK = SCAN_POS_PER_THREAD * SCAN_THREADS;
constexpr int CELL_PAD = 64;
constexpr int GROUP_ALIGN = SCAN_POS_PER_BLOCK;
constexpr int MAX_ATTEMPTS = 10000;

constexpr uint8_t T_NONE = 0x00, T_INS = 0x10, T_SUB = 0x20, T_DEL = 0x30, TMASK = 0x30, BTMASK = 0x3f;

struct Event {
    int32_t  pos;
    uint8_t  type;
    uint8_t  hap;
    uint8_t  base;
    uint8_t  live;
    uint32_t len;
    uint32_t seg;
};

struct SegTab { const int32_t *start; const int32_t *len; const uint32_t *cindex; int32_t n; };

struct HapDev {
    uint8_t *cells;
    const uint8_t *view;
    int32_t *ins_pos;
    uint32_t *ins_len;
    uint32_t *ins_off;
    uint8_t *ins_bases;
    uint32_t n_ins;
    int32_t pos_off;
};

struct ContigDev {
    HapDev hap[2];
    const uint8_t *ref;
    int64_t l;
    SegTab seg;
    const uint32_t *tot4;
    uint32_t cap_bases[2];
};

struct Count { const uint64_t *dev; uint32_t host; };

struct WalkParams {
    double mut_rate, indel_frac, indel_extend;
    uint64_t mut_thr;
    uint64_t gap_r; int32_t gap_s;
    const uint32_t *lg;
    int32_t indel_min, is_hap;
    uint32_t seed;
};

struct SimParams {
    double std_dev, mut_freq, rand_read, quality_std;
    int32_t dist, is_inner, len[2], max_n, strandedness, read_one_strand, amplicons, fixed_quality, data_type;
    int32_t has_bwa, has_bfast;
    uint32_t seed;
    float q_k, q_eps, q_lmin; int32_t q_near1;
};

inline uint64_t flow_ilog2_fixed(uint64_t y, int fb)
{
    const int p = 63 - __builtin_clzll(y);
    uint64_t m = y << (63 - p), frac = 0;
    for (int k = 0; k < fb; ++k) {
        const unsigned __int128 sq = (unsigned __int128)m * m;
        if ((uint64_t)(sq >> 127)) { m = (uint64_t)(sq >> 64); frac = (frac << 1) | 1u; }
        else { m = (uint64_t)(sq >> 63); frac <<= 1; }
    }
    return ((uint64_t)p << fb) | frac;
}
inline void flow_log2_table(uint32_t *lg)
{
    for (int i = 0; i < 256; ++i) lg[i] = (uint32_t)flow_ilog2_fixed(256u + (uint64_t)i, 32);
    lg[256] = 0xFFFFFFFFu;
}
inline void flow_gap_params(uint64_t thr, uint64_t *R, int32_t *s)
{
    *R = 0; *s = 0;
    if (thr == 0 || thr >= 0x100000000ull) return;
    const uint64_t Lq = (32ull << 56) - flow_ilog2_fixed(0x100000000ull - thr, 56);
    const int sh = __builtin_clzll(Lq);
    const unsigned __int128 q = ((unsigned __int128)1 << 127) / (Lq << sh);
    if ((uint64_t)(q >> 64)) { *R = 1ull << 63; *s = 62 - sh; }
    else { *R = (uint64_t)q; *s = 63 - sh; }
}

struct CalibArgs {
    uint32_t seed; int32_t end, len; uint64_t n_reads, first_read, chunk_reads;
    uint64_t thr;
    uint64_t gap_r; int32_t gap_s;
    const uint8_t *flow; int32_t flow_len, lds_words, stack_words;
    uint32_t *scratch;
    uint64_t *counters;
};

constexpr int SUMM_CELLS = 64;
constexpr int SUMM2_CELLS = 1024;

inline constexpr int flow_words_per_lane(int lds_words) { return lds_words | 1; }

struct SimSeg {
    uint32_t first_block;
    uint32_t contig_index;
    int32_t  start, l;
    uint64_t first_ii, n_pairs;
    uint64_t pair_off;
    int64_t  l_place;
    int32_t  reg_off, n_reg;
    uint32_t name_off; int32_t name_fixed_len;
    uint32_t contig_start;
    uint32_t pad_;
};

struct SimArgs {
    SimParams p;
    HapDev hap[2];
    const SimSeg *segs; int32_t n_seg; uint32_t n_blocks;
    uint64_t n_pairs;
    const uint64_t *chain;
    const int32_t *reg; int32_t have_regions;
    const uint64_t *e_thr[2];
    const uint16_t *summ[2];
    const uint16_t *summ2[2];
    int32_t place_fast, place_k;
    uint32_t *place_list, *place_list_n; uint32_t place_list_cap;
    uint64_t *range_rand;
    const uint32_t *e_thr32[2];
    int32_t e_full;
    const uint32_t *qbase[2];
    int32_t qb_words;
    const uint8_t *names;
    const uint8_t *rand_fixed; int32_t rand_fixed_len;
    uint32_t *meta;
    uint32_t *block_rand;
    uint64_t *counters;
    uint64_t *status[4];
    uint8_t *out[3];
    int32_t lds_words;
    int32_t cap;
    int32_t ion_lds;
    int32_t flow_stack_words;
    int32_t fifo;
    int32_t sim_threads;
    int32_t flow_len;
    int32_t split;
    uint32_t *split_state;
    uint32_t *split_hand;
    uint32_t *split_agg;
    uint64_t *split_pre;
    uint64_t *split_chunk;
    uint32_t *flow_scratch;
    uint64_t *flow_free;
    int32_t flow_slots;
    int32_t lb_shift;
    const uint8_t *flow;
    uint64_t flow_gap_r[2]; int32_t flow_gap_s[2];
    uint64_t err_thr_max[2], err_gap_r[2]; int32_t err_gap_s[2], err_ramp[2];
};

}
```

### dwgsim_amd/csrc/dw_launch.hpp

```cpp
#pragma once
#include <hip/hip_runtime.h>
#include "dw_kernels.hpp"

namespace dw {
void launch_pack(hipStream_t st, const uint8_t *ascii, uint8_t *ref, uint8_t *h0, uint8_t *h1, int64_t l);
void launch_site_scan_list(hipStream_t st, const uint8_t *refview, int64_t l, SegTab seg, WalkParams wp, uint64_t *status, uint64_t *ticket, int32_t *out, uint32_t cap, uint64_t *n_out);
uint32_t site_scan_blocks(int64_t l);
uint32_t site_scan_block_positions();
void launch_site_scan_slots(hipStream_t st, const uint8_t *refview, int64_t l, SegTab seg, WalkParams wp, int32_t *slots, uint32_t slot_cap, uint32_t *aux, int32_t *out, uint32_t cap, uint64_t *n_out, uint32_t *over);
void launch_mark_dirty(hipStream_t st, const Event *ev, Count n, const int32_t *lo, uint32_t *dirty);
void launch_dirty_chunks(hipStream_t st, bool restore, const uint32_t *dirty, uint32_t n_words, int64_t l_live, const uint8_t *ref, const uint8_t *refview, const uint16_t *refsumm, const uint16_t *refsumm2,
                         uint8_t *cells0, uint8_t *cells1, uint8_t *view0, uint8_t *view1, uint16_t *summ0, uint16_t *summ1, uint16_t *summ2_0, uint16_t *summ2_1);
void launch_scan_excl(hipStream_t st, uint32_t *data, uint32_t n, uint64_t *total_out);
void launch_compact(hipStream_t st, const uint16_t *mask, const uint32_t *block_base, int32_t *out, int64_t l, uint32_t cap);
void launch_events(hipStream_t st, const int32_t *cand, Count n, const uint8_t *ref, SegTab seg, WalkParams wp, Event *ev, uint32_t *max_del);
void walk_debug_seg_min(uint32_t rows);
void launch_resolve(hipStream_t st, Event *ev, Count n, const uint32_t *max_del, uint4 *flags, uint32_t *tot4);
void launch_apply(hipStream_t st, Event *ev, Count n, const uint4 *flags, ContigDev c, WalkParams wp);
void launch_justify_seq(hipStream_t st, const Event *ev, Count n, ContigDev c);
void launch_justify(hipStream_t st, const Event *ev, Count n, ContigDev c, int32_t *lo, int32_t *sufmin, uint8_t *bound);
void launch_mut_debug(hipStream_t st, const uint8_t *ref, const uint8_t *h0, const uint8_t *h1, int64_t l, uint64_t *verdict);
void launch_make_view(hipStream_t st, const uint8_t *cells0, const uint8_t *cells1, int64_t n_cells, int64_t l_live, uint8_t *view0, uint8_t *view1, uint16_t *summ0, uint16_t *summ1, uint16_t *summ2_0, uint16_t *summ2_1);
void launch_apply_patches(hipStream_t st, const int32_t *pos, const uint16_t *cells, uint32_t n, uint8_t *h0, uint8_t *h1);
void launch_collect_mask(hipStream_t st, const uint8_t *h0, const uint8_t *h1, int64_t l, uint16_t *mask, uint32_t *block_count);
void launch_gather(hipStream_t st, const int32_t *pos, uint32_t n, const uint8_t *ref, const uint8_t *h0, const uint8_t *h1, uint32_t *cells);
void launch_place(hipStream_t st, const SimArgs &a);
bool launch_simulate(hipStream_t st, const SimArgs &a, const SimForm &f);
void launch_calibrate(hipStream_t st, const CalibArgs &a);
void launch_failrule(hipStream_t st, const uint32_t *meta, uint64_t n_pairs, uint32_t opens_contig, uint64_t *summ, uint64_t *counters, uint64_t *chain);
void launch_chain_set(hipStream_t st, uint64_t *chain, uint64_t rand_base, int set_rand, uint64_t carry, int set_carry);
void launch_init(hipStream_t st, uint64_t *counters, uint32_t n_counters, uint64_t *z0, uint64_t n0, uint64_t *z1, uint64_t n1, uint64_t *chain, uint64_t rand_base, int set_rand, uint64_t carry, int set_carry);
void launch_selftest_lazy(hipStream_t st, int mode, uint32_t first, uint64_t n, double sigma, float qk, float qeps, float qlmin, int qnear1, uint64_t *out);
uint64_t gz_chunks(uint64_t n);
uint64_t gz_capacity(uint64_t n);
void gz_host_tables(uint32_t *crc_table, uint32_t *crc_shift);
void launch_gzip(hipStream_t st, const uint8_t *text, const uint64_t *n_dev, uint64_t text_cap, uint8_t *out, uint64_t out_cap, uint64_t *status, uint64_t *ticket, uint64_t *total, uint64_t *flags,
                 const uint32_t *crc_table, const uint32_t *crc_shift);
void launch_count_byte(hipStream_t st, const uint8_t *text, uint64_t n, uint32_t byte, uint64_t *out);
void launch_selftest_fp64(hipStream_t st, uint32_t seed, uint64_t n, uint64_t *mism);
void launch_selftest_text(hipStream_t st, uint64_t first, uint64_t n, uint64_t stride, uint64_t *out);
void launch_selftest_gap(hipStream_t st, const uint32_t *lg, uint64_t R, int sR, uint32_t first, uint64_t n, uint32_t g_lo, uint32_t g_cnt, uint32_t *chg, uint64_t *out);
}
```

### dwgsim_amd/csrc/dw_simulate.hip

```cpp
#include <algorithm>
#include "dw_read.hpp"
#include "dw_launch.hpp"

#ifndef DW_PART
#define DW_PART -1
#endif
#define DW_HAS(part) (DW_PART == -1 || DW_PART == (part))
#ifndef DW_SIM_WAVES
#define DW_SIM_WAVES 5
#endif
#ifndef DW_SOLID_WAVES
#define DW_SOLID_WAVES 4
#endif
#ifndef DW_SIM_WAVES_BOTH
#define DW_SIM_WAVES_BOTH 4
#endif
#ifndef DW_SIMB_WAVES
#define DW_SIMB_WAVES 6
#endif
#ifndef DW_IONA_WAVES
#define DW_IONA_WAVES 4
#endif
#ifndef DW_IONL_WAVES
#define DW_IONL_WAVES 3
#endif
#ifndef DW_ION_WAVES
#define DW_ION_WAVES 5
#endif

namespace dw {

#if DW_HAS(0)
DW_DEV bool attempt_surely_accepted(const uint16_t *summ, int64_t l, int64_t start, int step, int s)
{
    const int64_t far = start + (int64_t)step * (2 * (int64_t)s + 2);
    const int64_t lo = step > 0 ? start : far, hi = step > 0 ? far : start;
    if (lo < 0 || hi >= l) return false;
    uint32_t indel = 0, flags = 0;
    for (int64_t b = lo / SUMM_CELLS; b <= hi / SUMM_CELLS; ++b) { const uint32_t v = summ[b]; indel += v & 0xffu; flags |= v; }
    return !(flags & 0x8000u) && indel <= (uint32_t)s;
}

DW_DEV bool pair_surely_accepted(const SimArgs &a, const SegCtx &sc, RngKey key, uint64_t ii, uint32_t att, const U4 &b0)
{
    const int32_t s0 = a.p.len[0], s1 = a.p.len[1], smax = s0 > s1 ? s0 : s1, smin = s1 > 0 && s1 < s0 ? s1 : s0;
    const int64_t l = sc.l;
    if (l < (int64_t)s0 + s1 + 1 || sc.l_place != sc.l) return false;
    int64_t dlo = 0, dhi = 0;
    if (s1 > 0) {
        dlo = (int64_t)a.p.dist - a.place_k; dhi = (int64_t)a.p.dist + a.place_k;
        if (dlo < s0 + s1) dlo = s0 + s1;
        if (dhi < s0 + s1) dhi = s0 + s1;
        if (dlo > l) dlo = l;
        if (dhi > l) dhi = l;
    }
    const double u = u_lo(rng_block(key, D_PLACE, ii, att, 0, 0));
    const int64_t pos_lo = (int64_t)(int32_t)((double)(l - dhi + 1) * u), pos_hi = (int64_t)(int32_t)((double)(l - dlo + 1) * u);
    const int64_t lo = pos_lo - (2 * (int64_t)smax + 2), hi = pos_hi + dhi + s0 + s1 + 2 * (int64_t)smax + 2;
    if (lo < 0 || hi >= l) return false;
    const int hap = u_hi(b0) < a.p.mut_freq ? 0 : 1;
    const uint16_t *summ2 = (hap ? a.summ2[1] : a.summ2[0]) + sc.start / SUMM2_CELLS;
    uint32_t indel = 0, flags = 0;
    for (int64_t b = lo / SUMM2_CELLS; b <= hi / SUMM2_CELLS; ++b) { const uint32_t v = summ2[b]; indel += v & 0x7fffu; flags |= v; }
    return !(flags & 0x8000u) && indel <= (uint32_t)smin;
}

DW_DEV void place_pair_exact(const SimArgs &a, const SegCtx &sc, RngKey key, uint64_t ii, bool &is_rand, bool &failed, uint32_t &att)
{
    att = 0; is_rand = false; failed = false;
    for (;;) {
        const U4 b0 = rng_block(key, D_PAIR, ii, att, 0, 0);
        if (!(a.p.rand_read < u_lo(b0))) { is_rand = true; return; }
        if (a.place_fast && pair_surely_accepted(a, sc, key, ii, att, b0)) return;
        const PairDraw pd = draw_pair(a, sc, key, ii, att);
        if (pd.is_rand) { is_rand = true; return; }
        bool ok = true;
        for (int j = 0; j < 2 && ok; ++j) {
            const int sj = sel_len(a, j);
            if (sj <= 0) continue;
            int64_t start; int step;
            read_geom(a, sc, pd, j, &start, &step);
            if (!attempt_surely_accepted((pd.hap ? a.summ[1] : a.summ[0]) + sc.start / SUMM_CELLS, sc.l, start, step, sj)) {
                const ReadRes r = gen_read(sel_hap(a, sc, pd.hap), sc.l, start, step, sj, j ? pd.strand1 : pd.strand0, NoSink{});
                ok = r.ext_coor >= 0 && r.num_n <= a.p.max_n;
            }
        }
        if (ok) return;
        if (++att > (uint32_t)MAX_ATTEMPTS) { failed = true; return; }
    }
}

__global__ void __launch_bounds__(PLACE_PAIRS) k_place(SimArgs a)
{
    __shared__ uint32_t s_cnt[PLACE_PAIRS / 64];
    const int tid = (int)threadIdx.x, lane = tid & 63, wave = tid >> 6;
    const SegPtr sg = as_constant(a.segs) + seg_of_block(as_constant(a.segs), a.n_seg, blockIdx.x);
    const SegCtx sc = seg_ctx(a, sg);
    const uint64_t pair = (uint64_t)(blockIdx.x - sg->first_block) * PLACE_PAIRS + (uint64_t)tid;
    const bool valid = pair < sg->n_pairs;
    const uint64_t ii = sg->first_ii + pair;
    const RngKey key{a.p.seed, uniform_u32(sg->contig_index)};
    bool is_rand = false, open = false;
    if (valid) {
        const U4 b0 = rng_block(key, D_PAIR, ii, 0, 0, 0);
        is_rand = !(a.p.rand_read < u_lo(b0));
        open = !is_rand && !(a.place_fast && pair_surely_accepted(a, sc, key, ii, 0, b0));
    }
    const uint64_t rm = __ballot(is_rand), om = __ballot(open);
    if (lane == 0) s_cnt[wave] = (uint32_t)__popcll(rm);
    if (om) {
        const uint32_t li = (blockIdx.x * (PLACE_PAIRS / 64) + (uint32_t)wave) % PLACE_LISTS;
        uint32_t base = 0;
        if (lane == 0) base = atomicAdd(&a.place_list_n[16 * li], (uint32_t)__popcll(om));
        base = (uint32_t)__shfl((int)base, 0);
        const uint32_t at = base + (uint32_t)__popcll(om & ((1ull << lane) - 1ull));
        if (open) {
            if (at < a.place_list_cap) a.place_list[(size_t)li * a.place_list_cap + at] = blockIdx.x * (uint32_t)PLACE_PAIRS + (uint32_t)tid;
            else atomicOr((unsigned long long *)&a.counters[2], 16ull);
        }
    }
    __syncthreads();
    if (tid == 0) { uint32_t t = 0; for (int w = 0; w < PLACE_PAIRS / 64; ++w) t += s_cnt[w]; a.block_rand[blockIdx.x] = t; }
}

__global__ void __launch_bounds__(128) k_place_rest(SimArgs a)
{
    const int lane = (int)(threadIdx.x & 63);
    const uint32_t li = blockIdx.x % PLACE_LISTS, sub = blockIdx.x / PLACE_LISTS, nsub = gridDim.x / PLACE_LISTS;
    uint32_t n = a.place_list_n[16 * li];
    if (n > a.place_list_cap) n = a.place_list_cap;
    for (uint32_t base = sub * 128u; base < n; base += nsub * 128u) {
        const uint32_t q = base + threadIdx.x;
        bool todo = q < n;
        uint32_t e = 0, myseg = 0;
        if (todo) { e = a.place_list[(size_t)li * a.place_list_cap + q]; myseg = seg_of_block(as_constant(a.segs), a.n_seg, e / PLACE_PAIRS); }
        uint32_t retries = 0;
        for (;;) {
            const uint64_t m = __ballot(todo);
            if (!m) break;
            const uint32_t s = uniform_u32((uint32_t)__shfl((int)myseg, __ffsll((unsigned long long)m) - 1));
            if (todo && myseg == s) {
                const SegPtr sg = as_constant(a.segs) + s;
                const SegCtx sc = seg_ctx(a, sg);
                const uint64_t pair = (uint64_t)(e / PLACE_PAIRS - sg->first_block) * PLACE_PAIRS + (uint64_t)(e % PLACE_PAIRS);
                const RngKey key{a.p.seed, uniform_u32(sg->contig_index)};
                bool is_rand, failed; uint32_t att;
                place_pair_exact(a, sc, key, sg->first_ii + pair, is_rand, failed, att);
                if (is_rand) atomicAdd((unsigned long long *)&a.range_rand[s], 1ull);
                if (failed) atomicOr((unsigned long long *)&a.counters[2], 1ull);
                retries = att;
                todo = false;
            }
        }
        const uint32_t rs = wave_sum_u32(retries);
        if (lane == 0 && rs) atomicAdd((unsigned long long *)&a.counters[1], (unsigned long long)rs);
    }
}

__global__ void __launch_bounds__(256) k_range_counts(SimArgs a)
{
    const uint32_t q = blockIdx.x * 256u + threadIdx.x;
    if (q >= (uint32_t)a.n_seg) return;
    const SegPtr sg = as_constant(a.segs);
    const uint64_t lo = a.block_rand[sg[q].first_block], hi = q + 1 < (uint32_t)a.n_seg ? (uint64_t)a.block_rand[sg[q + 1].first_block] : a.counters[3];
    a.range_rand[q] += hi - lo;
    if (q == 0) { uint64_t open = 0; for (int li = 0; li < PLACE_LISTS; ++li) open += a.place_list_n[16 * li]; a.counters[5] = open; }
}
#endif


template <class O>
DW_DEV void put_name_fixed(O &o, const uint32_t *fw, const uint8_t *fx, uint32_t fixed_len)
{
    const uint32_t flen = fixed_len + 1, inl = flen < 128u ? flen : 128u;
    uint32_t q = 0;
    for (; q + 4 <= inl; q += 4) o.put4(fw[q >> 2]);
    if (q < inl) o.putn((uint64_t)fw[q >> 2] & ((1ull << (8 * (inl - q))) - 1), inl - q);
    for (q = inl; q < flen; ++q) o.put(fx[q]);
}
template <class O>
DW_DEV void put_rand_tail(O &o, uint64_t rand_ii)
{
    o.putn(0x305F305F305F305Full, 8);
    o.putn(0x3A305F315F315F00ull >> 8, 7);
    o.putn(0x303A305F303A30ull, 7);
    o.putn(0x303Aull, 2);
    put_hex(o, rand_ii, '_');
}
struct NameCounts { int32_t e0, u0, i0, e1, u1, i1; };
template <class O>
DW_DEV void put_pair_tail(O &o, int32_t x0, int32_t x1, uint32_t strand0, uint32_t strand1, const NameCounts &n, uint64_t ii)
{
    put_dec(o, (uint32_t)(x0 + 1), '_'); put_dec(o, (uint32_t)(x1 + 1), '_');
    o.putn((uint64_t)'_' | ((uint64_t)('0' + strand0) << 8) | ((uint64_t)'_' << 16) | ((uint64_t)('0' + strand1) << 24)
               | ((uint64_t)'_' << 32) | ((uint64_t)'0' << 40) | ((uint64_t)'_' << 48) | ((uint64_t)'0' << 56), 8);
    put_counts(o, (uint32_t)n.e0, (uint32_t)n.u0, (uint32_t)n.i0);
    put_counts(o, (uint32_t)n.e1, (uint32_t)n.u1, (uint32_t)n.i1);
    put_hex(o, ii, '_');
}
DW_DEV uint32_t pair_tail_len(int32_t x0, int32_t x1, const NameCounts &n, uint64_t ii)
{
    return 1 + ndigits10((uint32_t)(x0 + 1)) + 1 + ndigits10((uint32_t)(x1 + 1)) + 8
         + counts_len((uint32_t)n.e0, (uint32_t)n.u0, (uint32_t)n.i0) + counts_len((uint32_t)n.e1, (uint32_t)n.u1, (uint32_t)n.i1) + 1 + ndigits16(ii);
}
DW_DEV void quality_try_exact(uint32_t w, double sigma, bool &ok, int32_t &k0, int32_t &k1)
{
    const double v1 = (double)((int32_t)(w & 0xFFFFu) - 32768) * 0x1p-15, v2 = (double)((int32_t)(w >> 16) - 32768) * 0x1p-15;
    const double rsq = v1 * v1 + v2 * v2;
    ok = !(rsq >= 1.0 || rsq == 0.0);
    if (!ok) return;
    const double fac = sqrt_mid(div_mid(-2.0 * det_log<true>(rsq), rsq));
    k0 = (int32_t)(((v2 * fac) * sigma) + 0.5);
    k1 = (int32_t)(((v1 * fac) * sigma) + 0.5);
}
DW_DEV uint64_t quality_try_exact_called(uint32_t w, double sigma)
{
    bool ok; int32_t k0 = 0, k1 = 0;
    quality_try_exact(w, sigma, ok, k0, k1);
    return (uint64_t)(uint32_t)k0 | ((uint64_t)(uint32_t)k1 << 32);
}
struct QualLazy { float k, eps, lmin; int32_t near1_zero; };
DW_DEV uint32_t quality_try_lazy(uint32_t w, const QualLazy &ql, int32_t &k0, int32_t &k1)
{
    const uint32_t wx = w ^ 0x80008000u;
    const int32_t s1 = (int32_t)(int16_t)(wx & 0xFFFFu), s2 = (int32_t)wx >> 16;
    const uint32_t R = (uint32_t)(s1 * s1) + (uint32_t)(s2 * s2);
    const bool acc = R - 1u < 0x3FFFFFFFu;
    const float Rf = (float)R, rt = Rf * 0x1p-30f;
    const float Lp = -__builtin_amdgcn_logf(rt);
    const float f = __builtin_amdgcn_sqrtf(Lp * __builtin_amdgcn_rcpf(Rf));
// ... 54 lines not shown
        return;
    }
    const QualLazy ql{p.q_k, p.q_eps, p.q_lmin, p.q_near1};
    int pos = 0; uint32_t t = 0;
    while (pos < n_chars) {
        const U4 b = rng_block(key, dom, ii, att, 0, t++);
        uint64_t blk;
        const uint32_t nb = quality_block(b, ql, p.quality_std, qbw, nq, pos, blk);
        deliver(blk, nb, pos);
        pos += (int)nb;
    }
}

DW_DEV uint64_t hex_digits_sum(uint64_t b, uint64_t c)
{
    uint64_t sum = 0;
    for (int d = 1; d <= 16 && c; ++d) {
        const uint64_t hi = d == 16 ? ~0ull : (1ull << (4 * d)) - 1ull;
        if (b > hi) continue;
        const uint64_t n = hi - b + 1ull < c && d < 16 ? hi - b + 1ull : c;
        sum += n * (uint64_t)d; b += n; c -= n;
    }
    return sum;
}
DW_DEV uint32_t scratch_slot_take(uint64_t *ff, uint32_t per_xcd, uint32_t n_blocks)
{
    const uint32_t x = xcc_id();
    const uint64_t q = (uint64_t)atomicAdd((unsigned long long *)&ff[32 * x], 1ull);
    if (q < per_xcd) return x * per_xcd + (uint32_t)q;
    uint64_t *e = ff + 256 + (size_t)x * n_blocks + (size_t)(q - per_xcd);
    uint64_t v;
    do { v = status_load(e); if (v == 0) __builtin_amdgcn_s_sleep(2); } while (v == 0);
    return (uint32_t)(v - 1);
}
DW_DEV void scratch_slot_release(uint64_t *ff, uint32_t n_blocks, uint32_t slot)
{
    const uint32_t x = xcc_id();
    const uint64_t r = (uint64_t)atomicAdd((unsigned long long *)&ff[32 * x + 16], 1ull);
    status_store(ff + 256 + (size_t)x * n_blocks + (size_t)r, (uint64_t)slot + 1ull);
}
constexpr int sim_min_waves(int OUT, int DT, int NTHR, int WR, int SPLIT)
{
    if (DT == 3) return SPLIT == 1 ? DW_IONA_WAVES : SPLIT == 2 ? DW_SIMB_WAVES : DW_IONL_WAVES;
    if (NTHR != SIM_THREADS) return DT == 1 ? DW_SOLID_WAVES : 1;
    if (DT == 2) return DW_ION_WAVES;
    if (DT == 1) return DW_SOLID_WAVES;
    if (SPLIT == 2) return DW_SIMB_WAVES;
    return (OUT != 3 || WR != 0) ? DW_SIM_WAVES : DW_SIM_WAVES_BOTH;
}
template <int LPP, int OUT, int DT, int NTHR, int WR, int SPLIT>
__global__ void __launch_bounds__(NTHR, sim_min_waves(OUT, DT, NTHR, WR, SPLIT)) k_simulate(SimArgs a)
{
    static_assert(SPLIT == 0 || ((DT == 0 || DT == 3) && NTHR == SIM_THREADS), "the two-kernel form exists for the Illumina variants and for Ion Torrent with its buffers in LDS, 256-lane blocks");
    DW_DYN_SHARED(uint32_t, dyn_lds);
    __shared__ uint32_t sm_all[4][16];
    uint32_t (*const sm_bytes)[16] = sm_all, (*const sm_rand)[16] = sm_all + 3, (*const sm_one)[16] = sm_all;
    __shared__ uint32_t s_ticket, s_slot;
    __shared__ uint64_t s_rbase, s_base[3];
    __shared__ uint32_t s_fixed[2][32];
    __shared__ FlowTables s_ft;
    __shared__ uint32_t s_lg[FLOW_LG_ENTRIES];
    constexpr int nthr = NTHR, PPB = NTHR / LPP, nwaves = NTHR / 64;
    constexpr bool ION = DT == 2 || DT == 3;
    constexpr bool GS = DT == 2 || (DT != 3 && NTHR != SIM_THREADS);
    constexpr bool ONE_LB = (DT == 0 || DT == 1) && SPLIT == 0;
    const int LB_SHIFT = a.lb_shift;
    const int tid = (int)threadIdx.x;
    const int wave = tid >> 6, lane = tid & 63;
    DW_PROBE_INIT();
    if (GS && tid == 0) { s_slot = scratch_slot_take(a.flow_free, (uint32_t)a.flow_slots, a.n_blocks); asm volatile("" ::: "memory"); }
    if (SPLIT == 0 && tid == 0) s_ticket = (uint32_t)atomicAdd((unsigned long long *)&a.counters[0], 1ull);
    if (SPLIT != 1) for (int q = tid; q < 32; q += nthr) s_fixed[1][q] = reinterpret_cast<const uint32_t *>(a.rand_fixed)[q];
    if (ION && tid < 64) s_ft.flow[tid] = a.flow[tid];
    if (!ION && SPLIT != 2) for (int q = tid; q < FLOW_LG_ENTRIES; q += nthr) s_lg[q] = reinterpret_cast<const uint32_t *>(a.flow + 64)[q];
    const size_t stage_words = SPLIT == 2 ? 0 : DT == 3 ? (size_t)(a.lds_words + a.flow_stack_words) : DT == 2 ? (size_t)a.flow_stack_words : GS ? 0 : (size_t)a.lds_words;
    uint32_t *const s_qb = dyn_lds + stage_words * nthr;
    if (SPLIT != 1) for (int q = tid; q < 2 * a.qb_words; q += nthr) s_qb[q] = (q < a.qb_words ? a.qbase[0] : a.qbase[1])[q < a.qb_words ? q : q - a.qb_words];
    uint8_t *const s_fifo = reinterpret_cast<uint8_t *>(dyn_lds + (((stage_words * nthr + 2 * (size_t)a.qb_words) + 3) & ~(size_t)3)) + (size_t)tid * (WR == 2 ? SIM_FIFO_BYTES_WIDE : SIM_FIFO_BYTES);
    if (SPLIT == 0 || (SPLIT == 1 && !ION)) __syncthreads();
    constexpr int H = SPLIT;
    const uint32_t t = SPLIT == 0 ? uniform_u32(s_ticket) : (uint32_t)blockIdx.x;
    const SegPtr sg = as_constant(a.segs) + seg_of_block(as_constant(a.segs), a.n_seg, t);
    const SegCtx sc = seg_ctx(a, sg);
    const uint8_t *name_fixed = a.names + sg->name_off;
    if (H != 1) for (int q = tid; q < 32; q += nthr) s_fixed[0][q] = reinterpret_cast<const uint32_t *>(name_fixed)[q];
    if (ION) { if (SPLIT != 0) __syncthreads(); fill_flow_tables(s_ft, a.flow_len, tid, nthr, a.flow); __syncthreads(); }
    const int j = (LPP == 2) ? (tid & 1) : 0;
    const uint64_t pair_in = (uint64_t)(t - sg->first_block) * PPB + (uint64_t)(tid / LPP);
    const bool valid = pair_in < sg->n_pairs;
    const uint64_t ii = sg->first_ii + pair_in;
    const uint64_t pair = sg->pair_off + pair_in;
    const RngKey key{a.p.seed, uniform_u32(sg->contig_index)};
    const int s = sel_len(a, j);
    uint32_t *lds = GS ? a.flow_scratch + (size_t)uniform_u32(s_slot) * ((size_t)(DT == 2 ? flow_words_per_lane(a.lds_words) : a.lds_words) * nthr) + tid
                  : SPLIT == 2 ? a.split_state + (size_t)t * ((size_t)a.lds_words * nthr) + tid : dyn_lds + tid;
    uint32_t *const flow_stk = dyn_lds + (DT == 3 ? (size_t)a.lds_words * nthr : 0) + tid;
    const int capb = 16 * a.lds_words;

    if (SPLIT == 0) wave_priority(1);
    DW_PROBE_MARK(a, 0);
    PairDraw pd; pd.is_rand = true; pd.pos = pd.d = 0; pd.hap = 0; pd.strand0 = pd.strand1 = 0;
    ReadRes rr{0, 0, 0, 0, 0};
    uint32_t att = 0; bool is_rand = false, done = !valid;
    int32_t n_err = 0;
    int s_out = s;
    bool flow_reversed = false;
    const int nw = (s + 7) >> 3;
    int32_t err_first = 0;
    uint32_t rrank = 0, rtot = 0;
    uint32_t rb[4] = {0, 0, 0, 0};
    if (H != 2) {
    while (__ballot(!done)) {
        bool ok = true;
        if (!done) {
            pd = draw_pair(a, sc, key, ii, att);
            if (pd.is_rand) { is_rand = true; done = true; rr = ReadRes{0, 0, 0, 0, 0}; }
            else if (s > 0) {
                int64_t start; int step;
                read_geom(a, sc, pd, j, &start, &step);
                DW_PROBE_MARK(a, 7);
                if (ION) {
                    const bool rev = (j ? pd.strand1 : pd.strand0) != 0;
                    rr = gen_read(sel_hap(a, sc, pd.hap), sc.l, start, step, s, rev ? 1 : 0, FlowSink{lds, nthr, rev ? (capb >> 3) - 1 : ((capb - s) & ~7) >> 3, rev});
                }
                else if (probe::off(8)) { rr = ReadRes{(int32_t)start, 0, 0, 0, 0}; for (int w = 0; w * 8 < s; ++w) lds[w * nthr] = 0x32103210u; }
                else
                rr = gen_read(sel_hap(a, sc, pd.hap), sc.l, start, step, s, j ? pd.strand1 : pd.strand0, WordSink{lds, nthr});
                ok = rr.ext_coor >= 0 && rr.num_n <= a.p.max_n;
            }
        }
        if (LPP == 2) { const int other = __shfl_xor((int)ok, 1); ok = ok && (other != 0); }
        if (!done) {
            if (ok) done = true;
            else if (++att > (uint32_t)MAX_ATTEMPTS) { atomicOr((unsigned long long *)&a.counters[2], 1ull); done = true; }
        }
    }
    DW_PROBE_MARKF(a, 5);
    if (valid && j == 0) a.meta[pair] = att | (is_rand ? 0x80000000u : 0u) | ((sg->contig_start && pair_in == 0) ? 0x40000000u : 0u);
    { const uint32_t retries = wave_sum_u32((valid && j == 0) ? att : 0u); if (lane == 0 && retries) atomicAdd((unsigned long long *)&a.counters[1], (unsigned long long)retries); }
    if (H == 0 && !ONE_LB) {
    { const uint32_t v[1] = {(is_rand && j == 0) ? 1u : 0u}; uint32_t ex[1], tot[1]; block_excl_scan_n<1>(v, sm_rand, ex, tot); rrank = ex[0]; rtot = tot[0]; }
    DW_PROBE_MARKF(a, 6);
    if (wave == 0) {
        const uint64_t g = probe::off(128) ? (uint64_t)t * 6 : lookback_excl(a.status[2], t, rtot, 0);
        if (lane == 0) { s_rbase = g; if (t + 1 == a.n_blocks) a.counters[3] = g + rtot; }
    }
    }
    DW_PROBE_MARK(a, 1);
    if (ION) {
        const bool flows = valid && !is_rand && s > 0;
        FlowRng rg; rg.seed = key.seed; rg.contig = key.contig; rg.dom = D_FLOW0 + (uint32_t)j; rg.att = att; rg.evt = 0; rg.s = 0; rg.ii = ii; rg.w0 = rg.w1 = rg.w2 = rg.w3 = 0;
        const int so = flow_errors(flows, rg, s_ft, a.flow_len, (j ? a.e_thr[1] : a.e_thr[0])[0], j ? a.flow_gap_r[1] : a.flow_gap_r[0], j ? a.flow_gap_s[1] : a.flow_gap_s[0], lds, flow_stk, nthr, 2 * a.flow_stack_words, s, j ? pd.strand1 : pd.strand0, capb, &n_err);
        if (flows) {
            s_out = so;
            if (s_out < 0) { atomicOr((unsigned long long *)&a.counters[2], 2ull); s_out = 0; }
            flow_reversed = (j ? pd.strand1 : pd.strand0) != 0;
        }
    }
    if (ION) {
        if (valid && is_rand) for (int w = 0; w * 16 < s; ++w) {
            if ((w & 3) == 0) { const U4 q0 = rng_block(key, D_BASE0 + (uint32_t)j, ii, att, 0, (uint32_t)(w >> 2)); rb[0] = q0.x; rb[1] = q0.y; rb[2] = q0.z; rb[3] = q0.w; }
            uint32_t pairs = (w & 2) ? ((w & 1) ? rb[3] : rb[2]) : ((w & 1) ? rb[1] : rb[0]);
            const int rem = s - 16 * w;
            if (rem < 16) pairs &= (1u << (2 * rem)) - 1u;
            lds[w * nthr] = pairs;
        }
    } else
    if (valid && !(probe::off(4))) {
        if (is_rand) {
            uint32_t prev_base = 0;
            for (int w = 0; w < nw; ++w) {
                if ((w & 7) == 0) { const U4 q0 = rng_block(key, D_BASE0 + (uint32_t)j, ii, att, 0, (uint32_t)(w >> 3)); rb[0] = q0.x; rb[1] = q0.y; rb[2] = q0.z; rb[3] = q0.w; }
                const uint32_t wd = ((w >> 1) & 2) ? (((w >> 1) & 1) ? rb[3] : rb[2]) : (((w >> 1) & 1) ? rb[1] : rb[0]);
                uint32_t word = pairs_to_nibbles((wd >> (16 * (w & 1))) & 0xFFFFu);
                const int rem = s - 8 * w;
                const uint32_t live = rem >= 8 ? 0xFFFFFFFFu : ((1u << (4 * rem)) - 1u);
                if (DT == 1) {
                    const uint32_t prevw = (word << 4) | prev_base;
                    prev_base = word >> 28;
                    word = (word ^ prevw) & 0x33333333u;
                }
                lds[w * nthr] = word & live;
            }
        } else {
            if (DT == 1) {
                uint32_t prev_base = 0;
                for (int w = 0; w < nw; ++w) {
                    uint32_t word = lds[w * nthr];
                    const uint32_t prevw = (word << 4) | prev_base;
                    prev_base = word >> 28;
                    const uint32_t n = (word | prevw) & 0x44444444u;
                    word = ((word ^ prevw) & 0x33333333u & ~((n >> 1) | (n >> 2))) | n;
                    const int rem = s - 8 * w;
                    lds[w * nthr] = rem >= 8 ? word : word & ((1u << (4 * rem)) - 1u);
                }
            }
            const uint64_t tmax = j ? a.err_thr_max[1] : a.err_thr_max[0], gR = j ? a.err_gap_r[1] : a.err_gap_r[0];
            const int gS = j ? a.err_gap_s[1] : a.err_gap_s[0]; const bool ramp = (j ? a.err_ramp[1] : a.err_ramp[0]) != 0;
            const uint64_t *thr64 = j ? a.e_thr[1] : a.e_thr[0];
            if (tmax) {
                uint32_t m = 0, S = 0, tw[4] = {0, 0, 0, 0}, sw[4] = {0, 0, 0, 0};
                for (;;) {
                    if ((m & 3u) == 0u) {
                        const U4 q0 = rng_block(key, D_BASE0 + (uint32_t)j, ii, att, 0, m >> 2); rb[0] = q0.x; rb[1] = q0.y; rb[2] = q0.z; rb[3] = q0.w;
                        if (ramp) { const U4 q1 = rng_block(key, D_BASE_REF0 + (uint32_t)j, ii, att, 0, m >> 2); tw[0] = q1.x; tw[1] = q1.y; tw[2] = q1.z; tw[3] = q1.w; }
                    }
                    const uint32_t k4 = m & 3u;
                    const uint32_t gw = (k4 & 2u) ? ((k4 & 1u) ? rb[3] : rb[2]) : ((k4 & 1u) ? rb[1] : rb[0]);
                    const uint32_t G = tmax >= 0x100000000ull ? 0u : geom_gap(gw, s_lg, gR, gS);
                    S = m ? S + 1u + G : G;
                    if (S >= (uint32_t)s) break;
                    if (k4 == 0u) { const U4 q2 = rng_block(key, D_SUB0 + (uint32_t)j, ii, att, 0, m >> 2); sw[0] = q2.x; sw[1] = q2.y; sw[2] = q2.z; sw[3] = q2.w; }
                    const int w = (int)(S >> 3), sh = 4 * (int)(S & 7u);
                    const uint32_t word = lds[w * nthr];
                    bool hit = ((word >> sh) & 4u) == 0u;
                    if (ramp && hit) {
                        const uint64_t ti = thr64[S];
                        const uint32_t w2 = (k4 & 2u) ? ((k4 & 1u) ? tw[3] : tw[2]) : ((k4 & 1u) ? tw[1] : tw[0]);
                        hit = ti >= tmax || (uint64_t)w2 * tmax < (ti << 32);
                    }
                    if (hit) {
                        const uint32_t rwd = (k4 & 2u) ? ((k4 & 1u) ? sw[3] : sw[2]) : ((k4 & 1u) ? sw[1] : sw[0]);
// ... 723 lines not shown
```

### dwgsim_amd/csrc/dw_walk.hip

```cpp
#include "dw_device.hpp"
#include "dw_launch.hpp"
#include <stdlib.h>

namespace dw {

__global__ void k_pack(const uint8_t *__restrict__ ascii, uint8_t *__restrict__ ref, uint8_t *__restrict__ h0,
                       uint8_t *__restrict__ h1, int64_t l)
{
    const int64_t nchunk = (l + 15) >> 4;
    for (int64_t ch = (int64_t)blockIdx.x * blockDim.x + threadIdx.x; ch < nchunk; ch += (int64_t)gridDim.x * blockDim.x) {
        const int64_t p0 = ch << 4;
        uint32_t w[4] = {0, 0, 0, 0};
        if (p0 + 16 <= l) {
            const uint4 v = *reinterpret_cast<const uint4 *>(ascii + p0);
            const uint32_t in[4] = {v.x, v.y, v.z, v.w};
#pragma unroll
            for (int q = 0; q < 4; ++q)
#pragma unroll
                for (int b = 0; b < 4; ++b) w[q] |= code_of_ascii((in[q] >> (8 * b)) & 0xff) << (8 * b);
        } else {
            for (int b = 0; b < 16; ++b) { const uint32_t c = (p0 + b < l) ? code_of_ascii(ascii[p0 + b]) : 4u; w[b >> 2] |= c << (8 * (b & 3)); }
        }
        const uint4 o = make_uint4(w[0], w[1], w[2], w[3]);
        *reinterpret_cast<uint4 *>(ref + p0) = o;
// ... 679 lines not shown
{
    if (!n.host) return;
    hipLaunchKernelGGL(k_jreach, dim3(cdiv(n.host, 256)), dim3(256), 0, st, ev, n, c, lo);
    if (n.host < g_walk_seg_min_rows) hipLaunchKernelGGL(k_sufmin, dim3(1), dim3(1024), 0, st, lo, n, sufmin, 0u, (int32_t *)nullptr);
    else {
        const uint32_t seglen = (n.host + WALK_SEGS - 1) / WALK_SEGS;
        hipLaunchKernelGGL(k_sufmin, dim3(WALK_SEGS), dim3(1024), 0, st, lo, n, sufmin, seglen, sufmin + n.host);
        hipLaunchKernelGGL(k_sufmin_fix, dim3(cdiv(n.host, 256)), dim3(256), 0, st, sufmin, n, seglen, (const int32_t *)(sufmin + n.host));
    }
    hipLaunchKernelGGL(k_jbound, dim3(cdiv(n.host, 256)), dim3(256), 0, st, ev, n, c, sufmin, bound);
    hipLaunchKernelGGL(k_jrun, dim3(cdiv(n.host, 64)), dim3(64), 0, st, ev, n, c, bound);
}
__global__ void __launch_bounds__(SCAN_THREADS) k_mut_debug(const uint8_t *__restrict__ ref, const uint8_t *__restrict__ h0, const uint8_t *__restrict__ h1, int64_t l, uint64_t *verdict)
{
    const int64_t first = ((int64_t)blockIdx.x * SCAN_THREADS + threadIdx.x) * SCAN_POS_PER_THREAD;
    if (first >= l) return;
    const uint4 a = *reinterpret_cast<const uint4 *>(h0 + first), b = *reinterpret_cast<const uint4 *>(h1 + first);
    if ((((a.x | a.y | a.z | a.w) | (b.x | b.y | b.z | b.w)) & 0x30303030u) == 0) return;
    const uint4 r = *reinterpret_cast<const uint4 *>(ref + first);
    const uint32_t aw[4] = {a.x, a.y, a.z, a.w}, bw[4] = {b.x, b.y, b.z, b.w}, rw[4] = {r.x, r.y, r.z, r.w};
    for (int q = 0; q < SCAN_POS_PER_THREAD && first + q < l; ++q) {
        const uint32_t c0 = (rw[q >> 2] >> (8 * (q & 3))) & 0xffu, c1 = (aw[q >> 2] >> (8 * (q & 3))) & 0xffu, c2 = (bw[q >> 2] >> (8 * (q & 3))) & 0xffu;
        if (c0 >= 4 || ((c1 & TMASK) == T_NONE && (c2 & TMASK) == T_NONE)) continue;
        uint32_t code = 0;
        if ((c1 & BTMASK) == (c2 & BTMASK)) { if ((c1 & TMASK) == T_SUB && (c0 & 3) == (c1 & 3)) code = 1; }
        else if ((c1 & TMASK) == T_SUB || (c2 & TMASK) == T_SUB) {
            if ((c1 & 3) == (c2 & 3)) code = 2;
            else if (!((c0 & 3) == (c1 & 3) || (c0 & 3) == (c2 & 3))) code = 3;
        }
        if (code) { atomicMin((unsigned long long *)verdict, ((unsigned long long)(first + q) << 8) | code); return; }
    }
}
void launch_mut_debug(hipStream_t st, const uint8_t *ref, const uint8_t *h0, const uint8_t *h1, int64_t l, uint64_t *verdict)
{
    if (l > 0) hipLaunchKernelGGL(k_mut_debug, dim3(cdiv((uint64_t)l, SCAN_POS_PER_BLOCK)), dim3(SCAN_THREADS), 0, st, ref, h0, h1, l, verdict);
}
__global__ void __launch_bounds__(256) k_make_view(const uint8_t *__restrict__ cells0, const uint8_t *__restrict__ cells1, int64_t n_cells, int64_t l_live, uint8_t *__restrict__ view0, uint8_t *__restrict__ view1,
                                                   uint16_t *__restrict__ summ0, uint16_t *__restrict__ summ1, uint16_t *__restrict__ summ2_0, uint16_t *__restrict__ summ2_1)
{
    const uint8_t *__restrict__ cells = blockIdx.y ? cells1 : cells0;
    uint8_t *__restrict__ view = blockIdx.y ? view1 : view0;
    uint16_t *__restrict__ summ = blockIdx.y ? summ1 : summ0, *__restrict__ summ2 = blockIdx.y ? summ2_1 : summ2_0;
    const int64_t t = (int64_t)blockIdx.x * 256 + threadIdx.x, first = t * 32;
    const bool live = first < n_cells;
    uint32_t out[4] = {0, 0, 0, 0}, indel = 0, non_acgt = 0;
    if (live) {
#pragma unroll
        for (int q = 0; q < 2; ++q) {
            if (first + 16 * q >= n_cells) break;
            const uint4 v = *reinterpret_cast<const uint4 *>(cells + first + 16 * q);
            const uint32_t w[4] = {v.x, v.y, v.z, v.w};
#pragma unroll
            for (int b = 0; b < 16; ++b) {
                const uint32_t c = (w[b >> 2] >> (8 * (b & 3))) & 0xffu, ty = c & TMASK, base = c & 0xfu;
                const uint32_t nib = ty == T_NONE ? (base < 4 ? base : base == 4 ? 8u : 9u) : (ty == T_SUB && base < 4) ? 4u + base : 15u;
                const int cell = 16 * q + b;
                out[cell >> 3] |= nib << (4 * (cell & 7));
            }
#pragma unroll
            for (int k = 0; k < 4; ++k) {
                const int64_t rem = l_live - (first + 16 * q + 4 * k);
                const uint32_t lm = rem >= 4 ? 0xFFFFFFFFu : rem <= 0 ? 0u : ((1u << (8 * (int)rem)) - 1u);
                indel += (uint32_t)__popc(w[k] & lm & 0x10101010u);
                non_acgt |= w[k] & lm & 0x0C0C0C0Cu;
            }
        }
        *reinterpret_cast<uint4 *>(view + (first >> 1)) = make_uint4(out[0], out[1], out[2], out[3]);
    }
    uint32_t i1 = indel, f1 = non_acgt ? 1u : 0u;
#pragma unroll
    for (int d = 1; d < SUMM_CELLS / 32; d <<= 1) { i1 += (uint32_t)__shfl_xor((int)i1, d); f1 |= (uint32_t)__shfl_xor((int)f1, d); }
    uint32_t i2 = i1, f2 = f1;
#pragma unroll
    for (int d = SUMM_CELLS / 32; d < SUMM2_CELLS / 32; d <<= 1) { i2 += (uint32_t)__shfl_xor((int)i2, d); f2 |= (uint32_t)__shfl_xor((int)f2, d); }
    if (first < l_live) {
        if ((t & (SUMM_CELLS / 32 - 1)) == 0) summ[t / (SUMM_CELLS / 32)] = (uint16_t)(i1 | (f1 ? 0x8000u : 0u));
        if ((t & (SUMM2_CELLS / 32 - 1)) == 0) summ2[t / (SUMM2_CELLS / 32)] = (uint16_t)(i2 | (f2 ? 0x8000u : 0u));
    }
}
void launch_make_view(hipStream_t st, const uint8_t *cells0, const uint8_t *cells1, int64_t n_cells, int64_t l_live, uint8_t *view0, uint8_t *view1, uint16_t *summ0, uint16_t *summ1, uint16_t *summ2_0, uint16_t *summ2_1)
{
    if (n_cells > 0) hipLaunchKernelGGL(k_make_view, dim3(cdiv((uint64_t)n_cells, 256 * 32), 2), dim3(256), 0, st, cells0, cells1, n_cells, l_live, view0, view1, summ0, summ1, summ2_0, summ2_1);
}
void launch_apply_patches(hipStream_t st, const int32_t *pos, const uint16_t *cells, uint32_t n, uint8_t *h0, uint8_t *h1)
{
    if (n) hipLaunchKernelGGL(k_apply_patches, dim3(cdiv(n, 256)), dim3(256), 0, st, pos, cells, n, h0, h1);
}
void launch_collect_mask(hipStream_t st, const uint8_t *h0, const uint8_t *h1, int64_t l, uint16_t *mask, uint32_t *block_count)
{
    hipLaunchKernelGGL(k_collect_mask, dim3(cdiv((uint64_t)l, SCAN_POS_PER_BLOCK)), dim3(SCAN_THREADS), 0, st, h0, h1, l, mask, block_count);
}
void launch_gather(hipStream_t st, const int32_t *pos, uint32_t n, const uint8_t *ref, const uint8_t *h0, const uint8_t *h1, uint32_t *cells)
{
    if (n) hipLaunchKernelGGL(k_gather, dim3(cdiv(n, 256)), dim3(256), 0, st, pos, n, ref, h0, h1, cells);
}

}
```

Baseline: 1426.

## Pre-reject read placements that fall inside long N runs

Adds a per-contig table of the longest N-only runs, built from the reference bitmap and then clipped against the mutated haplotype cells after each walk. The simulate kernels consult this table to discard a drawn pair whose read window lies entirely inside an N run, before the full per-base N count is done. The aim is to cut wasted attempt work and wave divergence on references with large N gaps. In exchange it adds extra kernels and a device copy per group and walk, plus a small per-attempt table scan.

```diff
diff --git a/dwgsim_amd/api.py b/dwgsim_amd/api.py
--- a/dwgsim_amd/api.py
+++ b/dwgsim_amd/api.py
@@ -271,6 +271,7 @@
     n_pairs: int = 0
     n_random: int = 0
     n_retries: int = 0
+    nrun_rejected: int = 0
     kernel_ms: float = 0.0
     sim_kernel_ms: float = 0.0
     walk_ms: float = 0.0
@@ -587,6 +588,7 @@
                 n_sim += b.n_pairs
             ctx.drop_contig(h0)
         res.flow_cap_mult = ctx.debug_get("flow_cap_mult")
+        res.nrun_rejected = ctx.debug_get("nrun_rejected")
     res.n_pairs = n_sim
     res.n_random = rand_ii
     res.mutations_txt = bytes(txt)
diff --git a/dwgsim_amd/csrc/dw_host.cpp b/dwgsim_amd/csrc/dw_host.cpp
--- a/dwgsim_amd/csrc/dw_host.cpp
+++ b/dwgsim_amd/csrc/dw_host.cpp
@@ -45,6 +45,7 @@
     std::vector<uint8_t> h_names; std::vector<int32_t> h_reg, h_seg;
     DevMem d_summ[2], d_summ2[2];
     DevMem d_refview, d_refsumm, d_refsumm2, d_dirty;
+    DevMem d_nmap, d_nrun_ref, d_nrun;
     DevEvent ev_walk, ev_walk0;
     HostMem h_wc;
 };
@@ -150,6 +151,7 @@
     int ion_lds = -1;
     int n_cu = 0; int flow_slots = 0;
     int64_t walk_cap = -1; bool phases = false; int writer = -1, force_threads = 0; int64_t place_cap = -1; uint64_t place_open = 0; double walk_us = 0, count_us = 0; int split = -1;
+    bool nrun_reject = true; uint64_t nrun_rejected = 0;
     int64_t sim_form = 0;
     int64_t walk_form = 0;
     hipEvent_t ev_cnt0 = nullptr, ev_cnt1 = nullptr;
@@ -792,6 +794,26 @@
     return upload_table(c, M.d_reg, M.h_reg, 64);
 }
 
+static size_t nrun_bytes(const Group &g) { return sizeof(int32_t) * 2 * NRUN_MAX * g.m.size(); }
+static int make_nruns(dwgsim_hip_ctx_t *c, Group &g)
+{
+    GroupMem &M = g.mem;
+    const int64_t n_cells = (int64_t)padded_cells(g) & ~(int64_t)15;
+    const size_t map_bytes = ((size_t)n_cells / (64 * NRUN_CHUNK) + 2) * sizeof(uint64_t);
+    HIPC(c, reserve(c, M.d_nmap, map_bytes, map_bytes)); HIPC(c, reserve(c, M.d_nrun_ref, nrun_bytes(g), nrun_bytes(g) + 4096)); HIPC(c, reserve(c, M.d_nrun, nrun_bytes(g), nrun_bytes(g) + 4096));
+    HIPC(c, hipMemsetAsync(M.d_nmap.get(), 0, map_bytes, c->walk_stream));
+    launch_nruns(c->walk_stream, M.d_ref.get(), n_cells, M.d_nmap.get<uint16_t>(), seg_tab(g), M.d_nrun_ref.get<int32_t>());
+    HIPC(c, hipGetLastError());
+    return 0;
+}
+static int clip_nruns(dwgsim_hip_ctx_t *c, const Group &g, hipStream_t st)
+{
+    const GroupMem &M = g.mem;
+    HIPC(c, hipMemcpyAsync(M.d_nrun.get(), M.d_nrun_ref.get(), nrun_bytes(g), hipMemcpyDeviceToDevice, st));
+    launch_nrun_clip(st, M.d_cells[0].get(), M.d_cells[1].get(), seg_tab(g), M.d_nrun_ref.get<int32_t>(), M.d_nrun.get<int32_t>());
+    return 0;
+}
+
 static int build_group(dwgsim_hip_ctx_t *c, Group &g, const uint8_t *const *ascii, const int64_t *lens, const int64_t *starts)
 {
     const int n = (int)g.m.size();
@@ -801,6 +823,7 @@
     if (const int rc = upload_sequence(c, n, ascii, lens, starts, g.total, padded, must_wait)) return rc;
     if (const int rc = make_pristine(c, g)) return rc;
     if (const int rc = upload_group_tables(c, g)) return rc;
+    if (const int rc = make_nruns(c, g)) return rc;
     if (c->has_mutin) for (int k = 0; k < n; ++k) resolve_mutation_input(c->mutin, g.m[(size_t)k].contig_index, ascii[k], lens[k], (uint32_t)c->prm.seed, c->prm.is_hap != 0, g.m[(size_t)k].rc);
     if (must_wait) HIPC(c, hipStreamSynchronize(c->walk_stream));
     return 0;
@@ -1046,6 +1069,7 @@
         dirty_chunks(st, false, g);
         g.dirty_any = true;
     }
+    if (const int rc = clip_nruns(c, g, st)) return rc;
     HIPC(c, hipGetLastError());
     return DWGSIM_HIP_OK;
 }
@@ -1401,6 +1425,7 @@
         s.first_ii = r[q].first_ii; s.n_pairs = r[q].n_pairs; s.pair_off = pairs; s.l_place = m.l_place;
         s.reg_off = m.reg_off; s.n_reg = m.n_reg; s.name_off = m.name_off; s.name_fixed_len = m.name_fixed_len;
         s.contig_start = r[q].first_ii == 0 ? 1u : 0u;
+        s.nrun_off = (uint32_t)(2 * NRUN_MAX * k);
         segs.push_back(s);
         pairs += r[q].n_pairs; blocks += (r[q].n_pairs + ppb - 1) / ppb;
         if (m.name_fixed_len > fmax) fmax = m.name_fixed_len;
@@ -1477,6 +1502,8 @@
     a.e_full = c->e_full;
     a.names = g.mem.d_names.get();
     a.summ[0] = g.mem.d_summ[0].get<uint16_t>(); a.summ[1] = g.mem.d_summ[1].get<uint16_t>(); a.summ2[0] = g.mem.d_summ2[0].get<uint16_t>(); a.summ2[1] = g.mem.d_summ2[1].get<uint16_t>();
+    const bool n_rejects = (p.length[0] > 0 && p.max_n < p.length[0]) || (p.length[1] > 0 && p.max_n < p.length[1]);
+    a.nrun = (c->nrun_reject && !c->has_mutin && n_rejects) ? g.mem.d_nrun.get<int32_t>() : nullptr;
     a.place_fast = (!c->has_regions && !p.amplicons && p.std_dev * 12.1 + 2.0 < 1e9) ? 1 : 0;
     a.place_k = a.place_fast ? (int32_t)ceil(p.std_dev * 12.1) + 2 : 0;
     a.rand_fixed = c->d_rand_fixed.get(); a.rand_fixed_len = c->rand_fixed_len;
@@ -1744,6 +1771,7 @@
     }
     if (h[2] & 8) { c->err = "dwgsim-hip: the gzip output buffer is too small for this text\n"; return DWGSIM_HIP_ERR_FAILED; }
     for (int t = 0; t < 3; ++t) { sl.out_bytes[t] = h[4 + t]; sl.gz_bytes[t] = h[24 + t]; }
+    c->nrun_rejected += h[7];
     if (c->phases) {
         uint64_t tot = 0; for (int k = 0; k < 8; ++k) tot += h[8 + k];
         fprintf(stderr, "[phases]");
@@ -1947,6 +1975,7 @@
     else if (!strcmp(key, "flow_slots")) c->flow_slots = (int)value;
     else if (!strcmp(key, "ion_lds")) c->ion_lds = (int)value;
     else if (!strcmp(key, "flow_cap")) c->flow_cap_forced = (int)value;
+    else if (!strcmp(key, "nrun_reject")) c->nrun_reject = value != 0;
     else { c->err = "unknown debug option"; return DWGSIM_HIP_ERR_ARG; }
     return DWGSIM_HIP_OK;
 }
@@ -1959,6 +1988,7 @@
     else if (!strcmp(key, "walk_us")) *value = (int64_t)c->walk_us;
     else if (!strcmp(key, "count_us")) *value = (int64_t)c->count_us;
     else if (!strcmp(key, "sim_form")) *value = c->sim_form;
+    else if (!strcmp(key, "nrun_rejected")) *value = (int64_t)c->nrun_rejected;
     else if (!strcmp(key, "walk_form")) *value = c->walk_form;
     else { c->err = "unknown debug value"; return DWGSIM_HIP_ERR_ARG; }
     return DWGSIM_HIP_OK;
diff --git a/dwgsim_amd/csrc/dw_kernels.hpp b/dwgsim_amd/csrc/dw_kernels.hpp
--- a/dwgsim_amd/csrc/dw_kernels.hpp
+++ b/dwgsim_amd/csrc/dw_kernels.hpp
@@ -36,6 +36,9 @@
 constexpr int CELL_PAD = 64;
 constexpr int GROUP_ALIGN = SCAN_POS_PER_BLOCK;
 constexpr int MAX_ATTEMPTS = 10000;
+constexpr int NRUN_MAX = 16;
+constexpr int NRUN_CHUNK = 64;
+constexpr int NRUN_MARGIN = 2;
 
 constexpr uint8_t T_NONE = 0x00, T_INS = 0x10, T_SUB = 0x20, T_DEL = 0x30, TMASK = 0x30, BTMASK = 0x3f;
 
@@ -141,7 +144,7 @@
     int32_t  reg_off, n_reg;
     uint32_t name_off; int32_t name_fixed_len;
     uint32_t contig_start;
-    uint32_t pad_;
+    uint32_t nrun_off;
 };
 
 struct SimArgs {
@@ -154,6 +157,7 @@
     const uint64_t *e_thr[2];
     const uint16_t *summ[2];
     const uint16_t *summ2[2];
+    const int32_t *nrun;
     int32_t place_fast, place_k;
     uint32_t *place_list, *place_list_n; uint32_t place_list_cap;
     uint64_t *range_rand;
diff --git a/dwgsim_amd/csrc/dw_launch.hpp b/dwgsim_amd/csrc/dw_launch.hpp
--- a/dwgsim_amd/csrc/dw_launch.hpp
+++ b/dwgsim_amd/csrc/dw_launch.hpp
@@ -21,6 +21,8 @@
 void launch_justify(hipStream_t st, const Event *ev, Count n, ContigDev c, int32_t *lo, int32_t *sufmin, uint8_t *bound);
 void launch_mut_debug(hipStream_t st, const uint8_t *ref, const uint8_t *h0, const uint8_t *h1, int64_t l, uint64_t *verdict);
 void launch_make_view(hipStream_t st, const uint8_t *cells0, const uint8_t *cells1, int64_t n_cells, int64_t l_live, uint8_t *view0, uint8_t *view1, uint16_t *summ0, uint16_t *summ1, uint16_t *summ2_0, uint16_t *summ2_1);
+void launch_nruns(hipStream_t st, const uint8_t *ref, int64_t n_cells, uint16_t *nmap, SegTab seg, int32_t *tab);
+void launch_nrun_clip(hipStream_t st, const uint8_t *cells0, const uint8_t *cells1, SegTab seg, const int32_t *tab, int32_t *eff);
 void launch_apply_patches(hipStream_t st, const int32_t *pos, const uint16_t *cells, uint32_t n, uint8_t *h0, uint8_t *h1);
 void launch_collect_mask(hipStream_t st, const uint8_t *h0, const uint8_t *h1, int64_t l, uint16_t *mask, uint32_t *block_count);
 void launch_gather(hipStream_t st, const int32_t *pos, uint32_t n, const uint8_t *ref, const uint8_t *h0, const uint8_t *h1, uint32_t *cells);
diff --git a/dwgsim_amd/csrc/dw_simulate.hip b/dwgsim_amd/csrc/dw_simulate.hip
--- a/dwgsim_amd/csrc/dw_simulate.hip
+++ b/dwgsim_amd/csrc/dw_simulate.hip
@@ -30,6 +30,31 @@
 
 namespace dw {
 
+typedef const DW_CONST_AS int32_t *NrunPtr;
+DW_DEV bool attempt_surely_rejected(NrunPtr tab, int64_t start, int s)
+{
+    const int64_t wlo = start - (s + NRUN_MARGIN), whi = start + (s + NRUN_MARGIN);
+    bool in = false;
+    for (int e = 0; e < NRUN_MAX; ++e) {
+        const int32_t lo = tab[2 * e], nhi = tab[2 * e + 1];
+        if (nhi == 0) break;
+        in |= wlo >= (int64_t)lo && whi < -(int64_t)nhi;
+    }
+    return in;
+}
+DW_DEV bool pair_surely_rejected(const SimArgs &a, const SegCtx &sc, NrunPtr tab, const PairDraw &pd)
+{
+    bool rej = false;
+    for (int j = 0; j < 2; ++j) {
+        const int sj = sel_len(a, j);
+        if (sj <= 0 || sj <= a.p.max_n) continue;
+        int64_t start; int step;
+        read_geom(a, sc, pd, j, &start, &step);
+        rej |= attempt_surely_rejected(tab, start, sj);
+    }
+    return rej;
+}
+
 #if DW_HAS(0)
 DW_DEV bool attempt_surely_accepted(const uint16_t *summ, int64_t l, int64_t start, int step, int s)
 {
@@ -65,7 +90,7 @@
     return !(flags & 0x8000u) && indel <= (uint32_t)smin;
 }
 
-DW_DEV void place_pair_exact(const SimArgs &a, const SegCtx &sc, RngKey key, uint64_t ii, bool &is_rand, bool &failed, uint32_t &att)
+DW_DEV void place_pair_exact(const SimArgs &a, const SegCtx &sc, NrunPtr nrun, RngKey key, uint64_t ii, bool &is_rand, bool &failed, uint32_t &att)
 {
     att = 0; is_rand = false; failed = false;
     for (;;) {
@@ -74,7 +99,7 @@
         if (a.place_fast && pair_surely_accepted(a, sc, key, ii, att, b0)) return;
         const PairDraw pd = draw_pair(a, sc, key, ii, att);
         if (pd.is_rand) { is_rand = true; return; }
-        bool ok = true;
+        bool ok = !(a.nrun && att < (uint32_t)MAX_ATTEMPTS && pair_surely_rejected(a, sc, nrun, pd));
         for (int j = 0; j < 2 && ok; ++j) {
             const int sj = sel_len(a, j);
             if (sj <= 0) continue;
@@ -145,7 +170,7 @@
                 const uint64_t pair = (uint64_t)(e / PLACE_PAIRS - sg->first_block) * PLACE_PAIRS + (uint64_t)(e % PLACE_PAIRS);
                 const RngKey key{a.p.seed, uniform_u32(sg->contig_index)};
                 bool is_rand, failed; uint32_t att;
-                place_pair_exact(a, sc, key, sg->first_ii + pair, is_rand, failed, att);
+                place_pair_exact(a, sc, as_constant(a.nrun) + sg->nrun_off, key, sg->first_ii + pair, is_rand, failed, att);
                 if (is_rand) atomicAdd((unsigned long long *)&a.range_rand[s], 1ull);
                 if (failed) atomicOr((unsigned long long *)&a.counters[2], 1ull);
                 retries = att;
@@ -366,6 +391,7 @@
     const uint32_t t = SPLIT == 0 ? uniform_u32(s_ticket) : (uint32_t)blockIdx.x;
     const SegPtr sg = as_constant(a.segs) + seg_of_block(as_constant(a.segs), a.n_seg, t);
     const SegCtx sc = seg_ctx(a, sg);
+    const NrunPtr nrun = as_constant(a.nrun) + sg->nrun_off;
     const uint8_t *name_fixed = a.names + sg->name_off;
     if (H != 1) for (int q = tid; q < 32; q += nthr) s_fixed[0][q] = reinterpret_cast<const uint32_t *>(name_fixed)[q];
     if (ION) { if (SPLIT != 0) __syncthreads(); fill_flow_tables(s_ft, a.flow_len, tid, nthr, a.flow); __syncthreads(); }
@@ -385,7 +411,7 @@
     DW_PROBE_MARK(a, 0);
     PairDraw pd; pd.is_rand = true; pd.pos = pd.d = 0; pd.hap = 0; pd.strand0 = pd.strand1 = 0;
     ReadRes rr{0, 0, 0, 0, 0};
-    uint32_t att = 0; bool is_rand = false, done = !valid;
+    uint32_t att = 0, n_tab = 0; bool is_rand = false, done = !valid;
     int32_t n_err = 0;
     int s_out = s;
     bool flow_reversed = false;
@@ -397,7 +423,11 @@
     while (__ballot(!done)) {
         bool ok = true;
         if (!done) {
-            pd = draw_pair(a, sc, key, ii, att);
+            for (;;) {
+                pd = draw_pair(a, sc, key, ii, att);
+                if (!a.nrun || pd.is_rand || att >= (uint32_t)MAX_ATTEMPTS || !pair_surely_rejected(a, sc, nrun, pd)) break;
+                ++att; ++n_tab;
+            }
             if (pd.is_rand) { is_rand = true; done = true; rr = ReadRes{0, 0, 0, 0, 0}; }
             else if (s > 0) {
                 int64_t start; int step;
@@ -422,6 +452,7 @@
     DW_PROBE_MARKF(a, 5);
     if (valid && j == 0) a.meta[pair] = att | (is_rand ? 0x80000000u : 0u) | ((sg->contig_start && pair_in == 0) ? 0x40000000u : 0u);
     { const uint32_t retries = wave_sum_u32((valid && j == 0) ? att : 0u); if (lane == 0 && retries) atomicAdd((unsigned long long *)&a.counters[1], (unsigned long long)retries); }
+    if (a.nrun) { const uint32_t nt = wave_sum_u32((valid && j == 0) ? n_tab : 0u); if (lane == 0 && nt) atomicAdd((unsigned long long *)&a.counters[7], (unsigned long long)nt); }
     if (H == 0 && !ONE_LB) {
     { const uint32_t v[1] = {(is_rand && j == 0) ? 1u : 0u}; uint32_t ex[1], tot[1]; block_excl_scan_n<1>(v, sm_rand, ex, tot); rrank = ex[0]; rtot = tot[0]; }
     DW_PROBE_MARKF(a, 6);
diff --git a/dwgsim_amd/csrc/dw_walk.hip b/dwgsim_amd/csrc/dw_walk.hip
--- a/dwgsim_amd/csrc/dw_walk.hip
+++ b/dwgsim_amd/csrc/dw_walk.hip
@@ -785,6 +785,95 @@
 {
     if (n_cells > 0) hipLaunchKernelGGL(k_make_view, dim3(cdiv((uint64_t)n_cells, 256 * 32), 2), dim3(256), 0, st, cells0, cells1, n_cells, l_live, view0, view1, summ0, summ1, summ2_0, summ2_1);
 }
+__global__ void __launch_bounds__(256) k_nmap(const uint8_t *__restrict__ ref, int64_t n_cells, uint16_t *__restrict__ nmap)
+{
+    const int64_t t = (int64_t)blockIdx.x * 256 + threadIdx.x, first = t * 16;
+    bool all_n = false;
+    if (first < n_cells) {
+        const uint4 v = *reinterpret_cast<const uint4 *>(ref + first);
+        all_n = v.x == 0x04040404u && v.y == 0x04040404u && v.z == 0x04040404u && v.w == 0x04040404u;
+    }
+    uint64_t m = __ballot(all_n);
+    m &= m >> 1; m &= m >> 2;
+    uint32_t bits = 0;
+#pragma unroll
+    for (int k = 0; k < 16; ++k) bits |= (uint32_t)((m >> (4 * k)) & 1ull) << k;
+    if (lane_id() == 0 && (t >> 6) * 1024 < n_cells) nmap[t >> 6] = (uint16_t)bits;
+}
+
+__global__ void __launch_bounds__(64) k_nruns(const uint64_t *__restrict__ nmap, SegTab seg, int32_t *__restrict__ tab)
+{
+    const int lane = lane_id();
+    const uint32_t k = blockIdx.x;
+    const int64_t len = seg.len[k], w_first = seg.start[k] / (64 * NRUN_CHUNK), n_words = (len + 64 * NRUN_CHUNK - 1) / (64 * NRUN_CHUNK);
+    uint32_t t_len = 0; int32_t t_lo = 0;
+    bool open = false; int64_t run_start = 0;
+    auto close = [&](int64_t end_chunk) {
+        const int64_t lo = run_start * NRUN_CHUNK, hi = end_chunk * NRUN_CHUNK < len ? end_chunk * NRUN_CHUNK : len;
+        const uint32_t L = hi > lo ? (uint32_t)(hi - lo) : 0u;
+        uint64_t key = lane < NRUN_MAX ? ((uint64_t)t_len << 8 | (uint64_t)lane) : ~0ull;
+#pragma unroll
+        for (int d = 1; d < 64; d <<= 1) {
+            const uint64_t o = (uint64_t)(uint32_t)__shfl_xor((int)(uint32_t)key, d) | (uint64_t)(uint32_t)__shfl_xor((int)(uint32_t)(key >> 32), d) << 32;
+            key = o < key ? o : key;
+        }
+        if (L > (uint32_t)(key >> 8) && lane == (int)(key & 0xffu)) { t_len = L; t_lo = (int32_t)lo; }
+    };
+    for (int64_t w0 = 0; w0 < n_words; w0 += 64) {
+        const uint64_t mine = w0 + lane < n_words ? nmap[w_first + w0 + lane] : 0ull;
+        if (!__ballot(open ? mine != ~0ull : mine != 0ull)) continue;
+        for (int q = 0; q < 64 && w0 + q < n_words; ++q) {
+            const uint64_t x = (uint64_t)(uint32_t)__shfl((int)(uint32_t)mine, q) | (uint64_t)(uint32_t)__shfl((int)(uint32_t)(mine >> 32), q) << 32;
+            int pos = 0;
+            while (pos < 64) {
+                const uint64_t rest = (open ? ~x : x) >> pos;
+                if (!rest) break;
+                pos += __builtin_ctzll(rest);
+                const int64_t chunk = (w0 + q) * 64 + pos;
+                if (open) { close(chunk); open = false; } else { run_start = chunk; open = true; }
+            }
+        }
+    }
+    if (open) close(n_words * 64);
+    uint32_t rank = 0;
+    for (int q = 0; q < NRUN_MAX; ++q) {
+        const uint32_t ol = (uint32_t)__shfl((int)t_len, q);
+        rank += (ol > t_len || (ol == t_len && q < lane)) ? 1u : 0u;
+    }
+    if (lane < NRUN_MAX) { int32_t *e = tab + 2 * ((size_t)NRUN_MAX * k + rank); e[0] = t_len ? t_lo : 0; e[1] = t_len ? -(t_lo + (int32_t)t_len) : 0; }
+}
+
+__global__ void __launch_bounds__(256) k_nrun_clip(const uint8_t *__restrict__ cells0, const uint8_t *__restrict__ cells1, SegTab seg, const int32_t *__restrict__ tab, int32_t *__restrict__ eff)
+{
+    const uint32_t e = blockIdx.x, k = e / NRUN_MAX;
+    const int64_t lo = tab[2 * e], hi = -(int64_t)tab[2 * e + 1], mid = lo + (hi - lo) / 2, g0 = seg.start[k];
+    if (hi <= lo) return;
+    int64_t new_lo = lo, new_hi = hi;
+    const int64_t p0 = (g0 + lo) >> 4, p1 = (g0 + hi - 1) >> 4;
+    for (int64_t p = p0 + (int64_t)blockIdx.y * 256 + threadIdx.x; p <= p1; p += (int64_t)gridDim.y * 256) {
+        const uint4 a = *reinterpret_cast<const uint4 *>(cells0 + 16 * p), b = *reinterpret_cast<const uint4 *>(cells1 + 16 * p);
+        const uint32_t wa[4] = {a.x, a.y, a.z, a.w}, wb[4] = {b.x, b.y, b.z, b.w};
+        if (((wa[0] & wa[1] & wa[2] & wa[3] & wb[0] & wb[1] & wb[2] & wb[3]) == 0x04040404u) && ((wa[0] | wa[1] | wa[2] | wa[3] | wb[0] | wb[1] | wb[2] | wb[3]) == 0x04040404u)) continue;
+        for (int q = 0; q < 16; ++q) {
+            const int64_t pos = 16 * p + q - g0;
+            const uint32_t ca = (wa[q >> 2] >> (8 * (q & 3))) & 0xffu, cb = (wb[q >> 2] >> (8 * (q & 3))) & 0xffu;
+            if (pos < lo || pos >= hi || (ca == 4u && cb == 4u)) continue;
+            if (pos < mid) new_lo = pos + 1 > new_lo ? pos + 1 : new_lo; else new_hi = pos < new_hi ? pos : new_hi;
+        }
+    }
+    if (new_lo != lo) atomicMax(reinterpret_cast<uint32_t *>(&eff[2 * e]), (uint32_t)new_lo);
+    if (new_hi != hi) atomicMax(reinterpret_cast<uint32_t *>(&eff[2 * e + 1]), (uint32_t)(int32_t)-new_hi);
+}
+void launch_nruns(hipStream_t st, const uint8_t *ref, int64_t n_cells, uint16_t *nmap, SegTab seg, int32_t *tab)
+{
+    if (n_cells <= 0 || seg.n <= 0) return;
+    hipLaunchKernelGGL(k_nmap, dim3(cdiv((uint64_t)n_cells, 256 * 16)), dim3(256), 0, st, ref, n_cells, nmap);
+    hipLaunchKernelGGL(k_nruns, dim3((uint32_t)seg.n), dim3(64), 0, st, reinterpret_cast<const uint64_t *>(nmap), seg, tab);
+}
+void launch_nrun_clip(hipStream_t st, const uint8_t *cells0, const uint8_t *cells1, SegTab seg, const int32_t *tab, int32_t *eff)
+{
+    if (seg.n > 0) hipLaunchKernelGGL(k_nrun_clip, dim3((uint32_t)seg.n * NRUN_MAX, 8), dim3(256), 0, st, cells0, cells1, seg, tab, eff);
+}
 void launch_apply_patches(hipStream_t st, const int32_t *pos, const uint16_t *cells, uint32_t n, uint8_t *h0, uint8_t *h1)
 {
     if (n) hipLaunchKernelGGL(k_apply_patches, dim3(cdiv(n, 256)), dim3(256), 0, st, pos, cells, n, h0, h1);
```

Measured after the change: 1442 (median of 6 runs). 1.01x the previous value.
